# SamGalanakis/FlowCompare

Measured on NVIDIA B200. Metric: cloud-pairs/sec for per-point log p(x|ctx), higher is better.
Workload: dtype fp16x3(f32-faithful)

## Files before the change

flowcompare_b200/csrc/attention_tc.cu:

```cuda
#include <cuda_fp16.h>
#include "common.cuh"
#include "gemm.cuh"
#include "tcgen05.cuh"
#include <atomic>
#include <cstdlib>
#include <mutex>
#include <vector>

namespace {

constexpr int AQ = 128;
constexpr int AK = 64;
constexpr int AD = 64;
#ifndef A_SPL
#define A_SPL 4
#endif
constexpr int A_THREADS = 96 + 128 * A_SPL;
constexpr int A_ATOM = 64 * 128;
constexpr int A_QBYTES = 2 * AQ * 128;
constexpr uint32_t C_S = 128, C_O = 384;
template <bool F16> struct ACfg {
    static constexpr int TILE = F16 ? 2 * A_ATOM : 4 * A_ATOM;
    static constexpr int STAGES = F16 ? 4 : 2;
    static constexpr int SMEM = A_QBYTES + 2 * STAGES * TILE + 1024;
    static constexpr uint32_t C_QHI = 0, C_QLO = F16 ? 32 : 64, C_PHI = 256, C_PLO = F16 ? 288 : 320;
};
constexpr float A_QS = 16.0f;

struct AttnTcParams {
    float* out; int ldo;
    int N, Nc, nblk;
    float scale;
    int debug;
    int dbg_loads;
};

__device__ __forceinline__ void tmem_st16(uint32_t taddr, const uint32_t* r) {
    asm volatile(
        "tcgen05.st.sync.aligned.32x32b.x16.b32 [%0], {%1,%2,%3,%4,%5,%6,%7,%8,%9,%10,%11,%12,%13,%14,%15,%16};"
        ::"r"(taddr), "r"(r[0]), "r"(r[1]), "r"(r[2]), "r"(r[3]), "r"(r[4]), "r"(r[5]), "r"(r[6]), "r"(r[7]), "r"(r[8]),
          "r"(r[9]), "r"(r[10]), "r"(r[11]), "r"(r[12]), "r"(r[13]), "r"(r[14]), "r"(r[15]) : "memory");
}
__device__ __forceinline__ void tmem_st8(uint32_t taddr, const uint32_t* r) {
    asm volatile(
        "tcgen05.st.sync.aligned.32x32b.x8.b32 [%0], {%1,%2,%3,%4,%5,%6,%7,%8};"
        ::"r"(taddr), "r"(r[0]), "r"(r[1]), "r"(r[2]), "r"(r[3]), "r"(r[4]), "r"(r[5]), "r"(r[6]), "r"(r[7]) : "memory");
}
__device__ __forceinline__ float ex2_approx(float x) {
    float y;
    asm("ex2.approx.ftz.f32 %0, %1;" : "=f"(y) : "f"(x));
    return y;
}
__device__ __forceinline__ uint32_t tf32_hi(float x) { return (__float_as_uint(x) + 0x1000u) & 0xffffe000u; }

__device__ __forceinline__ void issue_3xtf32(uint32_t d, uint32_t a_hi, uint32_t a_lo, const unsigned char* b_tile, uint32_t idesc) {
#pragma unroll
    for (int kk = 0; kk < 8; ++kk) {
        const uint32_t atom = (uint32_t)(kk >> 2) * A_ATOM;
        const uint64_t adv = (uint64_t)((kk & 3) * 32 >> 4);
        const uint64_t dbh = make_kmajor_sw128_desc(smem_u32(b_tile + atom)) + adv;
        const uint64_t dbl = make_kmajor_sw128_desc(smem_u32(b_tile + 2 * A_ATOM + atom)) + adv;
        umma_tf32_ts(d, a_lo + 8 * kk, dbh, idesc, kk != 0);
        umma_tf32_ts(d, a_hi + 8 * kk, dbl, idesc, 1);
        umma_tf32_ts(d, a_hi + 8 * kk, dbh, idesc, 1);
    }
}

__device__ __forceinline__ void issue_3xf16(uint32_t d, uint32_t a_hi, uint32_t a_lo, const unsigned char* b_tile, uint32_t idesc) {
#pragma unroll
    for (int kk = 0; kk < 4; ++kk) {
        const uint64_t adv = (uint64_t)(kk * 32 >> 4);
        const uint64_t dbh = make_kmajor_sw128_desc(smem_u32(b_tile)) + adv;
        const uint64_t dbl = make_kmajor_sw128_desc(smem_u32(b_tile + A_ATOM)) + adv;
        umma_f16_ts(d, a_lo + 8 * kk, dbh, idesc, kk != 0);
        umma_f16_ts(d, a_hi + 8 * kk, dbl, idesc, 1);
        umma_f16_ts(d, a_hi + 8 * kk, dbh, idesc, 1);
    }
}

__device__ unsigned long long fc_attn_dbg[16];
#ifndef A_PHASE_TIMERS
#define A_PHASE_TIMERS 0
#endif
#if A_PHASE_TIMERS
#define DBG_T(var) const long long var = p.debug ? clock64() : 0
#else
#define DBG_T(var) const long long var = 0
#endif

template <bool F16>
__global__ void __launch_bounds__(A_THREADS, 1)
attention_tc_kernel(const __grid_constant__ CUtensorMap mapQ, const __grid_constant__ CUtensorMap mapKhi,
                    const __grid_constant__ CUtensorMap mapKlo, const __grid_constant__ CUtensorMap mapVhi,
                    const __grid_constant__ CUtensorMap mapVlo, const AttnTcParams p) {
    constexpr int A_STAGES = ACfg<F16>::STAGES, A_TILE = ACfg<F16>::TILE;
    constexpr uint32_t C_QHI = ACfg<F16>::C_QHI, C_QLO = ACfg<F16>::C_QLO, C_PHI = ACfg<F16>::C_PHI, C_PLO = ACfg<F16>::C_PLO;
    static_assert(!F16 || A_SPL == 2 || A_SPL == 4, "the fp16 form packs 32 (16) dims / keys per thread into one 16 (8) column store");
    extern __shared__ unsigned char smem_raw[];
    __shared__ __align__(8) uint64_t bars[2 + 4 * A_STAGES + 12];
    __shared__ uint32_t tmem_base_slot;
    __shared__ float mx_sm[2][A_SPL][AQ];

    const uint32_t raw = smem_u32(smem_raw);
    unsigned char* smem = smem_raw + ((1024u - (raw & 1023u)) & 1023u);
    unsigned char* q_raw = smem;
    auto k_tile = [&](int s) { return smem + A_QBYTES + s * A_TILE; };
    auto v_tile = [&](int s) { return smem + A_QBYTES + (A_STAGES + s) * A_TILE; };
    uint64_t* qfull = bars;
    uint64_t* qready = bars + 1;
    uint64_t* kfull = bars + 2;
    uint64_t* kfree = kfull + A_STAGES;
    uint64_t* vfull = kfree + A_STAGES;
    uint64_t* vfree = vfull + A_STAGES;
    uint64_t* s_ready = vfree + A_STAGES;
    uint64_t* s_free = s_ready + 2;
    constexpr int NPB = F16 ? 2 : 1;
    uint64_t* p_ready = s_free + 2;
    uint64_t* p_free = p_ready + 2;
    uint64_t* o_ready = p_free + 2;
    uint64_t* o_free = o_ready + 2;

    const int warp = threadIdx.x >> 5, lane = threadIdx.x & 31;
    const int b = blockIdx.y;
    const int q0 = blockIdx.x * AQ;
    const int nblk = p.nblk;

    if (threadIdx.x == 0) {
        mbar_init(qfull, 1); mbar_init(qready, 128 * A_SPL);
        for (int s = 0; s < A_STAGES; ++s) { mbar_init(&kfull[s], 1); mbar_init(&kfree[s], 1); mbar_init(&vfull[s], 1); mbar_init(&vfree[s], 1); }
        for (int s = 0; s < 2; ++s) { mbar_init(&s_ready[s], 1); mbar_init(&s_free[s], 128 * A_SPL); mbar_init(&o_ready[s], 1); mbar_init(&o_free[s], 128 * A_SPL); }
        for (int s = 0; s < 2; ++s) { mbar_init(&p_ready[s], 128 * A_SPL); mbar_init(&p_free[s], 1); }
        asm volatile("fence.mbarrier_init.release.cluster;" ::: "memory");
    }
    if (warp == 1) {
        asm volatile("tcgen05.alloc.cta_group::1.sync.aligned.shared::cta.b32 [%0], %1;" ::"r"(smem_u32(&tmem_base_slot)), "n"(512));
        asm volatile("tcgen05.relinquish_alloc_permit.cta_group::1.sync.aligned;");
    }
    asm volatile("tcgen05.fence::before_thread_sync;" ::: "memory");
    __syncthreads();
    asm volatile("tcgen05.fence::after_thread_sync;" ::: "memory");
    const uint32_t tmem = tmem_base_slot;

    if (warp == 0) {
        if (lane == 0) {
            mbar_expect_tx(qfull, A_QBYTES);
            tma_load_2d(&mapQ, q_raw, qfull, 0, b * p.N + q0);
            tma_load_2d(&mapQ, q_raw + AQ * 128, qfull, 32, b * p.N + q0);
            for (int i = 0; i < nblk; ++i) {
                const int s = i % A_STAGES;
                const uint32_t ph = (i / A_STAGES) & 1;
                const int krow = b * p.Nc + i * AK;
                mbar_wait(&kfree[s], ph ^ 1, 100 + i);
                if constexpr (F16) {
                    mbar_expect_tx(&kfull[s], A_TILE);
                    tma_load_2d(&mapKhi, k_tile(s), &kfull[s], 0, krow);
                    tma_load_2d(&mapKlo, k_tile(s) + A_ATOM, &kfull[s], 0, krow);
                    mbar_wait(&vfree[s], ph ^ 1, 150 + i);
                    mbar_expect_tx(&vfull[s], A_TILE);
                    tma_load_3d(&mapVhi, v_tile(s), &vfull[s], i * AK, 0, b);
                    tma_load_3d(&mapVlo, v_tile(s) + A_ATOM, &vfull[s], i * AK, 0, b);
                } else {
                mbar_expect_tx(&kfull[s], p.dbg_loads ? A_TILE / 2 : A_TILE);
                tma_load_2d(&mapKhi, k_tile(s), &kfull[s], 0, krow);
                tma_load_2d(&mapKhi, k_tile(s) + A_ATOM, &kfull[s], 32, krow);
                if (!p.dbg_loads) {
                tma_load_2d(&mapKlo, k_tile(s) + 2 * A_ATOM, &kfull[s], 0, krow);
                tma_load_2d(&mapKlo, k_tile(s) + 3 * A_ATOM, &kfull[s], 32, krow);
                }
                mbar_wait(&vfree[s], ph ^ 1, 150 + i);
                mbar_expect_tx(&vfull[s], p.dbg_loads ? A_TILE / 2 : A_TILE);
                tma_load_3d(&mapVhi, v_tile(s), &vfull[s], i * AK, 0, b);
                tma_load_3d(&mapVhi, v_tile(s) + A_ATOM, &vfull[s], i * AK + 32, 0, b);
                if (!p.dbg_loads) {
                tma_load_3d(&mapVlo, v_tile(s) + 2 * A_ATOM, &vfull[s], i * AK, 0, b);
                tma_load_3d(&mapVlo, v_tile(s) + 3 * A_ATOM, &vfull[s], i * AK + 32, 0, b);
                }
                }
            }
        }
    } else if (warp == 1) {
        const uint32_t idesc = (1u << 4) | ((F16 ? 0u : 2u) << 7) | ((F16 ? 0u : 2u) << 10) | ((uint32_t)(AK >> 3) << 17) | ((uint32_t)(AQ >> 4) << 24);
        long long w_kfull = 0, w_sfree = 0;
        DBG_T(t_start);
        mbar_wait(qready, 0, 200);
        asm volatile("tcgen05.fence::after_thread_sync;" ::: "memory");
        DBG_T(t_q);
        for (int j = 0; j < nblk; ++j) {
            const int ks = j % A_STAGES, sb = j & 1;
            DBG_T(c0);
            mbar_wait(&kfull[ks], (j / A_STAGES) & 1, 210 + j);
            DBG_T(c1);
            mbar_wait(&s_free[sb], ((j >> 1) & 1) ^ 1, 220 + j);
            DBG_T(c2);
            w_kfull += c1 - c0; w_sfree += c2 - c1;
            asm volatile("tcgen05.fence::after_thread_sync;" ::: "memory");
            if (elect_one()) {
                if constexpr (F16) issue_3xf16(tmem + C_S + 64 * sb, tmem + C_QHI, tmem + C_QLO, k_tile(ks), idesc);
                else issue_3xtf32(tmem + C_S + 64 * sb, tmem + C_QHI, tmem + C_QLO, k_tile(ks), idesc);
                umma_commit(&s_ready[sb]);
                umma_commit(&kfree[ks]);
            }
            __syncwarp();
        }
        if (A_PHASE_TIMERS && p.debug && lane == 0) {
            atomicAdd(&fc_attn_dbg[0], 1ull);
            atomicAdd(&fc_attn_dbg[1], (unsigned long long)(clock64() - t_start));
            atomicAdd(&fc_attn_dbg[2], (unsigned long long)w_kfull); atomicAdd(&fc_attn_dbg[3], (unsigned long long)w_sfree);
            atomicAdd(&fc_attn_dbg[11], (unsigned long long)(t_q - t_start));
        }
    } else if (warp == 2) {
        const uint32_t idesc = (1u << 4) | ((F16 ? 0u : 2u) << 7) | ((F16 ? 0u : 2u) << 10) | ((uint32_t)(AK >> 3) << 17) | ((uint32_t)(AQ >> 4) << 24);
        long long w_vfull = 0, w_ofree = 0, w_pready = 0;
        for (int i = 0; i < nblk; ++i) {
            const int vs = i % A_STAGES, ob = i & 1;
            DBG_T(c3);
            mbar_wait(&vfull[vs], (i / A_STAGES) & 1, 230 + i);
            DBG_T(c4);
            mbar_wait(&o_free[ob], ((i >> 1) & 1) ^ 1, 240 + i);
            DBG_T(c5);
            const int pb = NPB == 2 ? (i & 1) : 0;
            mbar_wait(&p_ready[pb], NPB == 2 ? (i >> 1) & 1 : i & 1, 250 + i);
            DBG_T(c6);
            w_vfull += c4 - c3; w_ofree += c5 - c4; w_pready += c6 - c5;
            asm volatile("tcgen05.fence::after_thread_sync;" ::: "memory");
            if (elect_one()) {
                if constexpr (F16) issue_3xf16(tmem + C_O + 64 * ob, tmem + C_PHI + 64 * pb, tmem + C_PLO + 64 * pb, v_tile(vs), idesc);
                else issue_3xtf32(tmem + C_O + 64 * ob, tmem + C_PHI, tmem + C_PLO, v_tile(vs), idesc);
                umma_commit(&o_ready[ob]);
                umma_commit(&p_free[pb]);
                umma_commit(&vfree[vs]);
            }
            __syncwarp();
        }
        if (A_PHASE_TIMERS && p.debug && lane == 0) {
            atomicAdd(&fc_attn_dbg[4], (unsigned long long)w_vfull); atomicAdd(&fc_attn_dbg[5], (unsigned long long)w_ofree);
            atomicAdd(&fc_attn_dbg[6], (unsigned long long)w_pready);
        }
    } else {
        constexpr int KS = AK / A_SPL;
        const int quad = warp & 3;
        const int sub = (warp - 3) >> 2;
        const int r = quad * 32 + lane;
        const uint32_t lane_addr = (uint32_t)(quad * 32) << 16;
        const int off = sub * KS;
        const float LOG2E = F16 ? 1.4426950408889634f / A_QS : 1.4426950408889634f;
        const int bar_id = 1 + quad;

        mbar_wait(qfull, 0, 300);
        if constexpr (F16) {
            uint32_t hi[KS / 2], lo[KS / 2];
            const unsigned char* atom = q_raw + (off >> 5) * (AQ * 128) + r * 128;
            const int j0 = (off & 31) >> 2;
            const float qs = p.scale * A_QS;
#pragma unroll
            for (int j = 0; j < KS / 4; ++j) {
                const float4 x = *reinterpret_cast<const float4*>(atom + (((j0 + j) ^ (r & 7)) << 4));
                const float xv[4] = {x.x * qs, x.y * qs, x.z * qs, x.w * qs};
#pragma unroll
                for (int e = 0; e < 4; e += 2) {
                    const uint32_t hp = pack_f16x2(xv[e], xv[e + 1]);
                    float h0, h1;
                    unpack_f16x2(hp, h0, h1);
                    hi[2 * j + (e >> 1)] = hp;
                    lo[2 * j + (e >> 1)] = pack_f16x2(xv[e] - h0, xv[e + 1] - h1);
                }
            }
            if constexpr (KS == 32) { tmem_st16(tmem + lane_addr + C_QHI + (off >> 1), hi); tmem_st16(tmem + lane_addr + C_QLO + (off >> 1), lo); }
            else                    { tmem_st8(tmem + lane_addr + C_QHI + (off >> 1), hi);  tmem_st8(tmem + lane_addr + C_QLO + (off >> 1), lo); }
        } else
#pragma unroll
        for (int c = 0; c < KS / 16; ++c) {
            uint32_t hi[16], lo[16];
            const int d0 = off + 16 * c;
            const unsigned char* atom = q_raw + (d0 >> 5) * (AQ * 128) + r * 128;
#pragma unroll
            for (int jj = 0; jj < 4; ++jj) {
                const int j = ((d0 & 31) >> 2) + jj;
                const float4 x = *reinterpret_cast<const float4*>(atom + ((j ^ (r & 7)) << 4));
                const float xv[4] = {x.x * p.scale, x.y * p.scale, x.z * p.scale, x.w * p.scale};
#pragma unroll
                for (int e = 0; e < 4; ++e) {
                    hi[4 * jj + e] = tf32_hi(xv[e]);
                    lo[4 * jj + e] = __float_as_uint(xv[e] - __uint_as_float(hi[4 * jj + e]));
                }
            }
            tmem_st16(tmem + lane_addr + C_QHI + d0, hi);
            tmem_st16(tmem + lane_addr + C_QLO + d0, lo);
        }
        asm volatile("tcgen05.wait::st.sync.aligned;" ::: "memory");
        asm volatile("tcgen05.fence::before_thread_sync;" ::: "memory");
        mbar_arrive(qready);

        float o[KS];
#pragma unroll
        for (int j = 0; j < KS; ++j) o[j] = 0.f;
        float m = -INFINITY, l = 0.f, alpha_prev = 0.f;

        auto load_cols = [&](uint32_t col, float (&dst)[KS]) {
#pragma unroll
            for (int c = 0; c < KS / 16; ++c) {
                uint32_t t16[16];
                tmem_ld16(tmem + lane_addr + col + 16 * c, t16);
#pragma unroll
                for (int j = 0; j < 16; ++j) dst[16 * c + j] = __uint_as_float(t16[j]);
            }
        };

        long long w_sready = 0, w_pfree = 0, w_oready = 0;
        DBG_T(t_sm0);
        for (int i = 0; i < nblk; ++i) {
            const int sb = i & 1;
            float sv[KS];
            DBG_T(d0);
            mbar_wait(&s_ready[sb], (i >> 1) & 1, 310 + i);
            DBG_T(d1);
            w_sready += d1 - d0;
            asm volatile("tcgen05.fence::after_thread_sync;" ::: "memory");
            load_cols(C_S + 64 * sb + off, sv);
            asm volatile("tcgen05.fence::before_thread_sync;" ::: "memory");
            mbar_arrive(&s_free[sb]);
            const int valid = p.Nc - i * AK - off;
            if (valid < KS) {
#pragma unroll
                for (int j = 0; j < KS; ++j) if (j >= valid) sv[j] = -INFINITY;
            }
            float mx4[4] = {sv[0], sv[1], sv[2], sv[3]};
#pragma unroll
            for (int j = 4; j < KS; ++j) mx4[j & 3] = fmaxf(mx4[j & 3], sv[j]);
            float mx = fmaxf(fmaxf(mx4[0], mx4[1]), fmaxf(mx4[2], mx4[3]));
            if (A_SPL > 1) {
                mx_sm[sb][sub][r] = mx;
                asm volatile("bar.sync %0, %1;" ::"r"(bar_id), "n"(32 * A_SPL) : "memory");
#pragma unroll
                for (int u = 0; u < A_SPL; ++u) mx = fmaxf(mx, mx_sm[sb][u][r]);
            }
            const float m_new = fmaxf(m, mx);
            const float alpha = ex2_approx((m - m_new) * LOG2E);
            const float mc = F16 ? fmaf(m_new, LOG2E, -10.0f) : m_new * LOG2E;
            float sum4[4] = {0.f, 0.f, 0.f, 0.f};
#pragma unroll
            for (int j = 0; j < KS; j += 4) {
                const float2 t0 = __ffma2_rn(make_float2(sv[j], sv[j + 1]), make_float2(LOG2E, LOG2E), make_float2(-mc, -mc));
                const float2 t1 = __ffma2_rn(make_float2(sv[j + 2], sv[j + 3]), make_float2(LOG2E, LOG2E), make_float2(-mc, -mc));
                sv[j] = ex2_approx(t0.x); sv[j + 1] = ex2_approx(t0.y); sv[j + 2] = ex2_approx(t1.x); sv[j + 3] = ex2_approx(t1.y);
                const float2 s01 = __fadd2_rn(make_float2(sum4[0], sum4[1]), make_float2(sv[j], sv[j + 1]));
                const float2 s23 = __fadd2_rn(make_float2(sum4[2], sum4[3]), make_float2(sv[j + 2], sv[j + 3]));
                sum4[0] = s01.x; sum4[1] = s01.y; sum4[2] = s23.x; sum4[3] = s23.y;
            }
            l = fmaf(l, alpha, (sum4[0] + sum4[1]) + (sum4[2] + sum4[3]));
            m = m_new;

            DBG_T(d2);
            const int pb = NPB == 2 ? (i & 1) : 0;
            mbar_wait(&p_free[pb], (NPB == 2 ? (i >> 1) & 1 : i & 1) ^ 1, 330 + i);
            DBG_T(d3);
            w_pfree += d3 - d2;
            asm volatile("tcgen05.fence::after_thread_sync;" ::: "memory");
            if constexpr (F16) {
                uint32_t hi[KS / 2], lo[KS / 2];
#pragma unroll
                for (int j = 0; j < KS / 2; ++j) {
                    const float p0 = sv[2 * j], p1 = sv[2 * j + 1];
                    const uint32_t hp = pack_f16x2(p0, p1);
                    float h0, h1;
                    unpack_f16x2(hp, h0, h1);
                    hi[j] = hp;
                    const float2 d2 = __fadd2_rn(make_float2(p0, p1), make_float2(-h0, -h1));
                    lo[j] = pack_f16x2(d2.x, d2.y);
                }
                if constexpr (KS == 32) { tmem_st16(tmem + lane_addr + C_PHI + 64 * pb + (off >> 1), hi); tmem_st16(tmem + lane_addr + C_PLO + 64 * pb + (off >> 1), lo); }
                else                    { tmem_st8(tmem + lane_addr + C_PHI + 64 * pb + (off >> 1), hi);  tmem_st8(tmem + lane_addr + C_PLO + 64 * pb + (off >> 1), lo); }
            } else
#pragma unroll
            for (int c = 0; c < KS / 16; ++c) {
                uint32_t hi[16], lo[16];
#pragma unroll
                for (int j = 0; j < 16; ++j) {
                    hi[j] = tf32_hi(sv[16 * c + j]);
                    lo[j] = __float_as_uint(sv[16 * c + j] - __uint_as_float(hi[j]));
                }
                tmem_st16(tmem + lane_addr + C_PHI + off + 16 * c, hi);
                tmem_st16(tmem + lane_addr + C_PLO + off + 16 * c, lo);
            }
            asm volatile("tcgen05.wait::st.sync.aligned;" ::: "memory");
            asm volatile("tcgen05.fence::before_thread_sync;" ::: "memory");
            mbar_arrive(&p_ready[pb]);

            if (i > 0) {
                const int ob = (i - 1) & 1;
                float ov[KS];
                DBG_T(d4);
                mbar_wait(&o_ready[ob], ((i - 1) >> 1) & 1, 350 + i);
                DBG_T(d5);
                w_oready += d5 - d4;
                asm volatile("tcgen05.fence::after_thread_sync;" ::: "memory");
                load_cols(C_O + 64 * ob + off, ov);
                asm volatile("tcgen05.fence::before_thread_sync;" ::: "memory");
                mbar_arrive(&o_free[ob]);
#pragma unroll
                for (int j = 0; j < KS; j += 2) {
                    const float2 o2 = __ffma2_rn(make_float2(o[j], o[j + 1]), make_float2(alpha_prev, alpha_prev), make_float2(ov[j], ov[j + 1]));
                    o[j] = o2.x; o[j + 1] = o2.y;
                }
            }
            alpha_prev = alpha;
        }
        if (A_PHASE_TIMERS && p.debug && threadIdx.x == 96) {
            atomicAdd(&fc_attn_dbg[7], (unsigned long long)w_sready); atomicAdd(&fc_attn_dbg[8], (unsigned long long)w_pfree);
            atomicAdd(&fc_attn_dbg[9], (unsigned long long)w_oready); atomicAdd(&fc_attn_dbg[10], (unsigned long long)(clock64() - t_sm0));
        }
        {
            const int ob = (nblk - 1) & 1;
            float ov[KS];
            mbar_wait(&o_ready[ob], ((nblk - 1) >> 1) & 1, 390);
            asm volatile("tcgen05.fence::after_thread_sync;" ::: "memory");
            load_cols(C_O + 64 * ob + off, ov);
#pragma unroll
            for (int j = 0; j < KS; ++j) o[j] = fmaf(o[j], alpha_prev, ov[j]);
        }
        if (A_SPL > 1) {
            mx_sm[nblk & 1][sub][r] = l;
            asm volatile("bar.sync %0, %1;" ::"r"(bar_id), "n"(32 * A_SPL) : "memory");
            l = 0.f;
#pragma unroll
            for (int u = 0; u < A_SPL; ++u) l += mx_sm[nblk & 1][u][r];
        }
        if (q0 + r < p.N) {
            const float inv = 1.0f / l;
            float4* dst = reinterpret_cast<float4*>(p.out + ((size_t)b * p.N + q0 + r) * p.ldo + off);
#pragma unroll
            for (int j = 0; j < KS / 4; ++j)
                dst[j] = make_float4(o[4 * j] * inv, o[4 * j + 1] * inv, o[4 * j + 2] * inv, o[4 * j + 3] * inv);
        }
    }
    asm volatile("tcgen05.fence::before_thread_sync;" ::: "memory");
    __syncthreads();
    if (warp == 1) {
        asm volatile("tcgen05.dealloc.cta_group::1.sync.aligned.b32 %0, %1;" ::"r"(tmem), "n"(512));
    }
}

template <bool F16>
__global__ void __launch_bounds__(256)
kv_split_kernel(const float* __restrict__ kv, int ldkv, int Nc, int Ncp, void* __restrict__ khi_, void* __restrict__ klo_,
                void* __restrict__ vthi_, void* __restrict__ vtlo_) {
    __shared__ float tile[32][AD + 1];
    const int b = blockIdx.y, key0 = blockIdx.x * 32, tid = threadIdx.x;
    auto put = [](void* hi_, void* lo_, size_t i, float x) {
        if (F16) {
            const __half h = __float2half_rn(x);
            static_cast<__half*>(hi_)[i] = h;
            static_cast<__half*>(lo_)[i] = __float2half_rn(x - __half2float(h));
        } else {
            const float h = __uint_as_float(tf32_hi(x));
            static_cast<float*>(hi_)[i] = h;
            static_cast<float*>(lo_)[i] = x - h;
        }
    };
    for (int idx = tid; idx < 32 * AD; idx += 256) {
        const int kk = idx >> 6, d = idx & 63;
        const int key = key0 + kk;
        if (key < Nc) {
            const float* src = kv + ((size_t)b * Nc + key) * ldkv;
            put(khi_, klo_, ((size_t)b * Nc + key) * AD + d, src[d]);
            tile[kk][d] = src[AD + d];
        } else {
            tile[kk][d] = 0.f;
        }
    }
    __syncthreads();
    for (int idx = tid; idx < 32 * AD; idx += 256) {
        const int d = idx >> 5, kk = idx & 31;
        const int key = key0 + kk;
        if (key < Ncp) put(vthi_, vtlo_, ((size_t)b * AD + d) * Ncp + key, tile[kk][d]);
    }
}

struct AMapKey {
    const void* base; uint64_t d0, d1, d2, s1, s2; uint32_t b0, b1; int f16;
    bool operator==(const AMapKey& o) const {
        return base == o.base && d0 == o.d0 && d1 == o.d1 && d2 == o.d2 && s1 == o.s1 && s2 == o.s2 && b0 == o.b0 && b1 == o.b1 && f16 == o.f16;
    }
};
std::vector<std::pair<AMapKey, CUtensorMap>> g_amaps;
std::mutex g_amaps_mu;

bool get_amap(const void* base, uint64_t d0, uint64_t d1, uint64_t d2, uint64_t s1, uint64_t s2, uint32_t b0, uint32_t b1,
              CUtensorMap* out, int f16 = 0) {
    AMapKey key{base, d0, d1, d2, s1, s2, b0, b1, f16};
    std::lock_guard<std::mutex> lk(g_amaps_mu);
    for (auto& kv : g_amaps) if (kv.first == key) { *out = kv.second; return true; }
    FcEncodeTiledFn enc = fc_get_encode_fn();
    if (!enc) return false;
    const cuuint32_t rank = d2 > 0 ? 3 : 2;
    cuuint64_t dims[3] = {d0, d1, d2 > 0 ? d2 : 1};
    const cuuint64_t esz = f16 ? 2 : 4;
    cuuint64_t strides[2] = {s1 * esz, s2 * esz};
    cuuint32_t box[3] = {b0, b1, 1};
    cuuint32_t estr[3] = {1, 1, 1};
    CUtensorMap m;
    if (enc(&m, f16 ? CU_TENSOR_MAP_DATA_TYPE_FLOAT16 : CU_TENSOR_MAP_DATA_TYPE_FLOAT32, rank, const_cast<void*>(base), dims, strides, box, estr,
            CU_TENSOR_MAP_INTERLEAVE_NONE, CU_TENSOR_MAP_SWIZZLE_128B, CU_TENSOR_MAP_L2_PROMOTION_L2_128B,
            CU_TENSOR_MAP_FLOAT_OOB_FILL_NONE) != CUDA_SUCCESS)
        return false;
    if (g_amaps.size() > 256) g_amaps.clear();
    g_amaps.emplace_back(key, m);
    *out = m;
    return true;
}

}

int64_t fc_attention_tc_scratch_floats(int B, int Nc) {
    const int64_t Ncp = fc_round_up(Nc, 8);
    return 2 * fc_round_up_ll((int64_t)B * Nc * AD, 32) + 2 * fc_round_up_ll((int64_t)B * AD * Ncp, 32) + 64;
}

void fc_attention_tc_scratch_layout(int B, int Nc, float* scratch, float** khi, float** klo, float** vthi, float** vtlo,
                                    int* ncp, int fmt) {
    const int Ncp = fc_round_up(Nc, fmt ? 8 : 4);
    *khi = scratch;
    *klo = *khi + fc_round_up_ll((int64_t)B * Nc * AD, 32);
    *vthi = *klo + fc_round_up_ll((int64_t)B * Nc * AD, 32);
    *vtlo = *vthi + fc_round_up_ll((int64_t)B * AD * fc_round_up(Nc, 8), 32);
    *ncp = Ncp;
}

namespace {
template <bool F16>
int launch_attention_tc(const float* q, int ldq, const float* kv, int ldkv, float* out, int ldo, int B, int N, int Nc, int d,
                        float scale, float* scratch, int presplit, cudaStream_t stream) {
    float *khi, *klo, *vthi, *vtlo;
    int Ncp;
    fc_attention_tc_scratch_layout(B, Nc, scratch, &khi, &klo, &vthi, &vtlo, &Ncp, F16 ? 1 : 0);
    CUtensorMap mQ, mKh, mKl, mVh, mVl;
    if (!get_amap(q, AD, (uint64_t)B * N, 0, (uint64_t)ldq, 0, 32, AQ, &mQ)) return FC_ERR_CUDA;
    const uint32_t bx = F16 ? 64 : 32;
    if (!get_amap(khi, AD, (uint64_t)B * Nc, 0, AD, 0, bx, AK, &mKh, F16)) return FC_ERR_CUDA;
    if (!get_amap(klo, AD, (uint64_t)B * Nc, 0, AD, 0, bx, AK, &mKl, F16)) return FC_ERR_CUDA;
    if (!get_amap(vthi, (uint64_t)Nc, AD, (uint64_t)B, (uint64_t)Ncp, (uint64_t)AD * Ncp, bx, AD, &mVh, F16)) return FC_ERR_CUDA;
    if (!get_amap(vtlo, (uint64_t)Nc, AD, (uint64_t)B, (uint64_t)Ncp, (uint64_t)AD * Ncp, bx, AD, &mVl, F16)) return FC_ERR_CUDA;
    int dev = 0;
    FC_CUDA_OK(cudaGetDevice(&dev));
    static std::atomic<uint64_t> configured{0};
    const uint64_t bit = 1ull << (dev & 63);
    if (!(configured.load(std::memory_order_acquire) & bit)) {
        FC_CUDA_OK(cudaFuncSetAttribute(attention_tc_kernel<F16>, cudaFuncAttributeMaxDynamicSharedMemorySize, ACfg<F16>::SMEM));
        configured.fetch_or(bit, std::memory_order_release);
    }
    FcProfScope prof(FC_CLS_ATTENTION, 4.0 * B * (double)N * Nc * d, 4.0 * B * ((double)N * d * 2 + (double)Nc * d * 2), stream);
    if (!presplit) {
        kv_split_kernel<F16><<<dim3((Ncp + 31) / 32, B), 256, 0, stream>>>(kv, ldkv, Nc, Ncp, khi, klo, vthi, vtlo);
        fc_count_launch();
    }
    static int dbg_loads = -1;
    if (dbg_loads < 0) { const char* e = getenv("FC_ATTN_DBG_LOADS"); dbg_loads = (e && e[0] == '1') ? 1 : 0; }
    static int dbg = -1;
    if (dbg < 0) { const char* e = getenv("FC_ATTN_DEBUG"); dbg = (e && e[0] == '1') ? 1 : 0; }
    AttnTcParams p{out, ldo, N, Nc, (Nc + AK - 1) / AK, scale, dbg, dbg_loads};
    attention_tc_kernel<F16><<<dim3((N + AQ - 1) / AQ, B), A_THREADS, ACfg<F16>::SMEM, stream>>>(mQ, mKh, mKl, mVh, mVl, p);
    fc_count_launch();
    FC_LAUNCH_OK();
    return FC_OK;
}
}

int fc_launch_cross_attention_tc(const float* q, int ldq, const float* kv, int ldkv, float* out, int ldo, int B, int N,
                                 int Nc, int d, float scale, float* scratch, int presplit, int fmt, cudaStream_t stream) {
    FC_REQUIRE(q && (kv || presplit) && out && scratch && B > 0 && N > 0 && Nc > 0);
    FC_REQUIRE((int64_t)B * N < (1ll << 31) - AQ && (int64_t)B * Nc < (1ll << 31) - AK);
    if (d != AD) return FC_ERR_UNSUPPORTED;
    FC_REQUIRE((ldq & 3) == 0 && (ldo & 3) == 0 && (presplit || ldkv >= 2 * AD) && ldq >= AD && ldo >= AD && B <= 65535);
    FC_REQUIRE((reinterpret_cast<uintptr_t>(q) & 15) == 0 && (reinterpret_cast<uintptr_t>(out) & 15) == 0 &&
               (reinterpret_cast<uintptr_t>(scratch) & 127) == 0);
    return fmt ? launch_attention_tc<true>(q, ldq, kv, ldkv, out, ldo, B, N, Nc, d, scale, scratch, presplit, stream)
               : launch_attention_tc<false>(q, ldq, kv, ldkv, out, ldo, B, N, Nc, d, scale, scratch, presplit, stream);
}

extern "C" __attribute__((visibility("default"))) int fc_debug_attn_phases(unsigned long long* out16) {
    if (cudaMemcpyFromSymbol(out16, fc_attn_dbg, 16 * sizeof(unsigned long long)) != cudaSuccess) return FC_ERR_CUDA;
    unsigned long long z[16] = {};
    if (cudaMemcpyToSymbol(fc_attn_dbg, z, sizeof(z)) != cudaSuccess) return FC_ERR_CUDA;
    return FC_OK;
}

extern "C" __attribute__((visibility("default"))) int64_t fc_cross_attention_tc_scratch_bytes(int B, int Nc) {
    if (B <= 0 || Nc <= 0) return FC_ERR_INVALID_ARG;
    return fc_attention_tc_scratch_floats(B, Nc) * 4;
}

extern "C" __attribute__((visibility("default"))) int fc_cross_attention_tc(const float* q, int ldq, const float* kv, int ldkv,
                                                                             float* out, int ldo, int B, int N, int Nc, int d,
                                                                             float scale, void* scratch, int64_t scratch_bytes,
                                                                             fc_stream_t stream) {
    FC_REQUIRE(scratch && scratch_bytes >= fc_cross_attention_tc_scratch_bytes(B, Nc));
    return fc_launch_cross_attention_tc(q, ldq, kv, ldkv, out, ldo, B, N, Nc, d, scale, static_cast<float*>(scratch), 0, 0,
                                        (cudaStream_t)stream);
}

extern "C" __attribute__((visibility("default"))) int fc_cross_attention_tc_f16(const float* q, int ldq, const float* kv, int ldkv,
                                                                                 float* out, int ldo, int B, int N, int Nc, int d,
                                                                                 float scale, void* scratch, int64_t scratch_bytes,
                                                                                 fc_stream_t stream) {
    FC_REQUIRE(scratch && scratch_bytes >= fc_cross_attention_tc_scratch_bytes(B, Nc));
    return fc_launch_cross_attention_tc(q, ldq, kv, ldkv, out, ldo, B, N, Nc, d, scale, static_cast<float*>(scratch), 0, 1,
                                        (cudaStream_t)stream);
}
```

flowcompare_b200/csrc/tcgen05.cuh:

```cuda
#pragma once
#include <cuda.h>
#include <cuda_runtime.h>
#include <cstdint>
#include <cstdio>

namespace {

__device__ __forceinline__ uint32_t smem_u32(const void* p) { return (uint32_t)__cvta_generic_to_shared(p); }

__device__ __forceinline__ void mbar_init(uint64_t* bar, uint32_t count) {
    asm volatile("mbarrier.init.shared::cta.b64 [%0], %1;" ::"r"(smem_u32(bar)), "r"(count));
}
__device__ __forceinline__ void mbar_expect_tx(uint64_t* bar, uint32_t bytes) {
    asm volatile("mbarrier.arrive.expect_tx.shared::cta.b64 _, [%0], %1;" ::"r"(smem_u32(bar)), "r"(bytes) : "memory");
}
__device__ __forceinline__ void mbar_arrive(uint64_t* bar) {
    asm volatile("mbarrier.arrive.shared::cta.b64 _, [%0];" ::"r"(smem_u32(bar)) : "memory");
}
__device__ __forceinline__ void mbar_timeout(int tag, uint32_t parity) {
    printf("flowcompare_b200 tcgen05 kernel: mbarrier wait timed out (tag %d, block %d,%d thread %d, parity %u)\n", tag,
           blockIdx.x, blockIdx.y, threadIdx.x, parity);
    __trap();
}
__device__ __forceinline__ void mbar_wait(uint64_t* bar, uint32_t parity, int tag = 0) {
    uint32_t done = 0;
    for (uint32_t spin = 0; spin < (1u << 22); ++spin) {
        asm volatile(
            "{\n\t"
            ".reg .pred p;\n\t"
            "mbarrier.try_wait.parity.shared::cta.b64 p, [%1], %2;\n\t"
            "selp.u32 %0, 1, 0, p;\n\t"
            "}" : "=r"(done) : "r"(smem_u32(bar)), "r"(parity) : "memory");
        if (done) return;
    }
    mbar_timeout(tag, parity);
}
__device__ __forceinline__ void mbar_wait_hint(uint64_t* bar, uint32_t parity, int tag, uint32_t hint_ns) {
    if (hint_ns == 0) { mbar_wait(bar, parity, tag); return; }
    uint32_t done = 0;
    for (uint32_t spin = 0; spin < (1u << 22); ++spin) {
        asm volatile(
            "{\n\t"
            ".reg .pred p;\n\t"
            "mbarrier.try_wait.parity.shared::cta.b64 p, [%1], %2, %3;\n\t"
            "selp.u32 %0, 1, 0, p;\n\t"
            "}" : "=r"(done) : "r"(smem_u32(bar)), "r"(parity), "r"(hint_ns) : "memory");
        if (done) return;
    }
    mbar_timeout(tag, parity);
}
__device__ __forceinline__ bool mbar_test(uint64_t* bar, uint32_t parity) {
    uint32_t done;
    asm volatile(
        "{\n\t"
        ".reg .pred p;\n\t"
        "mbarrier.test_wait.parity.shared::cta.b64 p, [%1], %2;\n\t"
        "selp.u32 %0, 1, 0, p;\n\t"
        "}" : "=r"(done) : "r"(smem_u32(bar)), "r"(parity) : "memory");
    return done != 0;
}
__device__ __forceinline__ void tma_load_2d(const CUtensorMap* map, void* smem_dst, uint64_t* bar, int c0, int c1) {
    asm volatile(
        "cp.async.bulk.tensor.2d.shared::cluster.global.mbarrier::complete_tx::bytes [%0], [%1, {%3, %4}], [%2];"
        ::"r"(smem_u32(smem_dst)), "l"(map), "r"(smem_u32(bar)), "r"(c0), "r"(c1) : "memory");
}
__device__ __forceinline__ void tma_load_2d_mcast(const CUtensorMap* map, void* smem_dst, uint64_t* bar, int c0, int c1,
                                                  uint16_t mask) {
    asm volatile(
        "cp.async.bulk.tensor.2d.shared::cluster.global.mbarrier::complete_tx::bytes.multicast::cluster"
        " [%0], [%1, {%3, %4}], [%2], %5;"
        ::"r"(smem_u32(smem_dst)), "l"(map), "r"(smem_u32(bar)), "r"(c0), "r"(c1), "h"(mask) : "memory");
}
__device__ __forceinline__ void tma_store_2d(const CUtensorMap* map, const void* smem_src, int c0, int c1) {
    asm volatile("cp.async.bulk.tensor.2d.global.shared::cta.bulk_group [%0, {%2, %3}], [%1];"
                 ::"l"(map), "r"(smem_u32(smem_src)), "r"(c0), "r"(c1) : "memory");
}
__device__ __forceinline__ void umma_commit(uint64_t* bar) {
    asm volatile("tcgen05.commit.cta_group::1.mbarrier::arrive::one.shared::cluster.b64 [%0];" ::"r"(smem_u32(bar)) : "memory");
}
__device__ __forceinline__ void umma_commit_mcast(uint64_t* bar, uint16_t mask) {
    asm volatile("tcgen05.commit.cta_group::1.mbarrier::arrive::one.shared::cluster.multicast::cluster.b64 [%0], %1;"
                 ::"r"(smem_u32(bar)), "h"(mask) : "memory");
}
__device__ __forceinline__ bool elect_one() {
    uint32_t pred;
    asm volatile("{\n\t.reg .b32 rx;\n\t.reg .pred px;\n\telect.sync rx|px, 0xffffffff;\n\tselp.u32 %0, 1, 0, px;\n\t}" : "=r"(pred));
    return pred != 0;
}
__device__ __forceinline__ void cluster_sync_all() {
    asm volatile("barrier.cluster.arrive.release.aligned;\n\tbarrier.cluster.wait.acquire.aligned;" ::: "memory");
}
__device__ __forceinline__ void umma_tf32_ts(uint32_t tmem_d, uint32_t tmem_a, uint64_t desc_b, uint32_t idesc, uint32_t accumulate) {
    #if !(defined(TC_KO_MMA) && TC_KO_MMA)
    asm volatile(
        "{\n\t"
        ".reg .pred p;\n\t"
        "setp.ne.b32 p, %4, 0;\n\t"
        "tcgen05.mma.cta_group::1.kind::tf32 [%0], [%1], %2, %3, p;\n\t"
        "}" ::"r"(tmem_d), "r"(tmem_a), "l"(desc_b), "r"(idesc), "r"(accumulate) : "memory");
#endif
}
__device__ __forceinline__ void umma_f16_ts(uint32_t tmem_d, uint32_t tmem_a, uint64_t desc_b, uint32_t idesc, uint32_t accumulate) {
    #if !(defined(TC_KO_MMA) && TC_KO_MMA)
    asm volatile(
        "{\n\t"
        ".reg .pred p;\n\t"
        "setp.ne.b32 p, %4, 0;\n\t"
        "tcgen05.mma.cta_group::1.kind::f16 [%0], [%1], %2, %3, p;\n\t"
        "}" ::"r"(tmem_d), "r"(tmem_a), "l"(desc_b), "r"(idesc), "r"(accumulate) : "memory");
#endif
}
__device__ __forceinline__ uint64_t make_kmajor_sw64_desc(uint32_t smem_addr) {
    uint64_t d = 0;
    d |= (uint64_t)((smem_addr & 0x3FFFF) >> 4);
    d |= (uint64_t)1 << 16;
    d |= (uint64_t)(512 >> 4) << 32;
    d |= (uint64_t)1 << 46;
    d |= (uint64_t)4 << 61;
    return d;
}
__device__ __forceinline__ uint32_t pack_f16x2(float lo_half, float hi_half) {
    uint32_t r;
    asm("cvt.rn.f16x2.f32 %0, %1, %2;" : "=r"(r) : "f"(hi_half), "f"(lo_half));
    return r;
}
__device__ __forceinline__ void unpack_f16x2(uint32_t v, float& lo_half, float& hi_half) {
    asm("{\n\t.reg .f16 l, h;\n\tmov.b32 {l, h}, %2;\n\tcvt.f32.f16 %0, l;\n\tcvt.f32.f16 %1, h;\n\t}" : "=f"(lo_half), "=f"(hi_half) : "r"(v));
}
__device__ __forceinline__ uint64_t make_kmajor_sw128_desc(uint32_t smem_addr) {
    uint64_t d = 0;
    d |= (uint64_t)((smem_addr & 0x3FFFF) >> 4);
    d |= (uint64_t)1 << 16;
    d |= (uint64_t)(1024 >> 4) << 32;
    d |= (uint64_t)1 << 46;
    d |= (uint64_t)2 << 61;
    return d;
}
__device__ __forceinline__ void tmem_ld16(uint32_t taddr, uint32_t (&r)[16]) {
    asm volatile(
        "tcgen05.ld.sync.aligned.32x32b.x16.b32 {%0,%1,%2,%3,%4,%5,%6,%7,%8,%9,%10,%11,%12,%13,%14,%15}, [%16];\n\t"
        "tcgen05.wait::ld.sync.aligned;"
        : "=r"(r[0]), "=r"(r[1]), "=r"(r[2]), "=r"(r[3]), "=r"(r[4]), "=r"(r[5]), "=r"(r[6]), "=r"(r[7]), "=r"(r[8]),
          "=r"(r[9]), "=r"(r[10]), "=r"(r[11]), "=r"(r[12]), "=r"(r[13]), "=r"(r[14]), "=r"(r[15])
        : "r"(taddr) : "memory");
}
__device__ __forceinline__ void tmem_ld16x2(uint32_t taddr_a, uint32_t taddr_b, uint32_t (&a)[16], uint32_t (&b)[16]) {
    asm volatile(
        "tcgen05.ld.sync.aligned.32x32b.x16.b32 {%0,%1,%2,%3,%4,%5,%6,%7,%8,%9,%10,%11,%12,%13,%14,%15}, [%32];\n\t"
        "tcgen05.ld.sync.aligned.32x32b.x16.b32 {%16,%17,%18,%19,%20,%21,%22,%23,%24,%25,%26,%27,%28,%29,%30,%31}, [%33];\n\t"
        "tcgen05.wait::ld.sync.aligned;"
        : "=r"(a[0]), "=r"(a[1]), "=r"(a[2]), "=r"(a[3]), "=r"(a[4]), "=r"(a[5]), "=r"(a[6]), "=r"(a[7]), "=r"(a[8]),
          "=r"(a[9]), "=r"(a[10]), "=r"(a[11]), "=r"(a[12]), "=r"(a[13]), "=r"(a[14]), "=r"(a[15]),
          "=r"(b[0]), "=r"(b[1]), "=r"(b[2]), "=r"(b[3]), "=r"(b[4]), "=r"(b[5]), "=r"(b[6]), "=r"(b[7]), "=r"(b[8]),
          "=r"(b[9]), "=r"(b[10]), "=r"(b[11]), "=r"(b[12]), "=r"(b[13]), "=r"(b[14]), "=r"(b[15])
        : "r"(taddr_a), "r"(taddr_b) : "memory");
}
__device__ __forceinline__ void tmem_ld16x2_issue(uint32_t taddr_a, uint32_t taddr_b, uint32_t (&a)[16], uint32_t (&b)[16]) {
    asm volatile(
        "tcgen05.ld.sync.aligned.32x32b.x16.b32 {%0,%1,%2,%3,%4,%5,%6,%7,%8,%9,%10,%11,%12,%13,%14,%15}, [%32];\n\t"
        "tcgen05.ld.sync.aligned.32x32b.x16.b32 {%16,%17,%18,%19,%20,%21,%22,%23,%24,%25,%26,%27,%28,%29,%30,%31}, [%33];"
        : "=r"(a[0]), "=r"(a[1]), "=r"(a[2]), "=r"(a[3]), "=r"(a[4]), "=r"(a[5]), "=r"(a[6]), "=r"(a[7]), "=r"(a[8]),
          "=r"(a[9]), "=r"(a[10]), "=r"(a[11]), "=r"(a[12]), "=r"(a[13]), "=r"(a[14]), "=r"(a[15]),
          "=r"(b[0]), "=r"(b[1]), "=r"(b[2]), "=r"(b[3]), "=r"(b[4]), "=r"(b[5]), "=r"(b[6]), "=r"(b[7]), "=r"(b[8]),
          "=r"(b[9]), "=r"(b[10]), "=r"(b[11]), "=r"(b[12]), "=r"(b[13]), "=r"(b[14]), "=r"(b[15])
        : "r"(taddr_a), "r"(taddr_b) : "memory");
}
__device__ __forceinline__ void tmem_ld16x2_wait(uint32_t (&a)[16], uint32_t (&b)[16]) {
    asm volatile("tcgen05.wait::ld.sync.aligned;"
        : "+r"(a[0]), "+r"(a[1]), "+r"(a[2]), "+r"(a[3]), "+r"(a[4]), "+r"(a[5]), "+r"(a[6]), "+r"(a[7]), "+r"(a[8]),
          "+r"(a[9]), "+r"(a[10]), "+r"(a[11]), "+r"(a[12]), "+r"(a[13]), "+r"(a[14]), "+r"(a[15]),
          "+r"(b[0]), "+r"(b[1]), "+r"(b[2]), "+r"(b[3]), "+r"(b[4]), "+r"(b[5]), "+r"(b[6]), "+r"(b[7]), "+r"(b[8]),
          "+r"(b[9]), "+r"(b[10]), "+r"(b[11]), "+r"(b[12]), "+r"(b[13]), "+r"(b[14]), "+r"(b[15])
        :: "memory");
}
__device__ __forceinline__ void tmem_st16(uint32_t taddr, const uint32_t (&r)[16]) {
    asm volatile(
        "tcgen05.st.sync.aligned.32x32b.x16.b32 [%0], {%1,%2,%3,%4,%5,%6,%7,%8,%9,%10,%11,%12,%13,%14,%15,%16};"
        ::"r"(taddr), "r"(r[0]), "r"(r[1]), "r"(r[2]), "r"(r[3]), "r"(r[4]), "r"(r[5]), "r"(r[6]), "r"(r[7]), "r"(r[8]),
          "r"(r[9]), "r"(r[10]), "r"(r[11]), "r"(r[12]), "r"(r[13]), "r"(r[14]), "r"(r[15]) : "memory");
}
__device__ __forceinline__ void tmem_st32(uint32_t taddr, const uint32_t (&r)[32]) {
    asm volatile(
        "tcgen05.st.sync.aligned.32x32b.x32.b32 [%0], {%1,%2,%3,%4,%5,%6,%7,%8,%9,%10,%11,%12,%13,%14,%15,%16,"
        "%17,%18,%19,%20,%21,%22,%23,%24,%25,%26,%27,%28,%29,%30,%31,%32};"
        ::"r"(taddr), "r"(r[0]), "r"(r[1]), "r"(r[2]), "r"(r[3]), "r"(r[4]), "r"(r[5]), "r"(r[6]), "r"(r[7]), "r"(r[8]),
          "r"(r[9]), "r"(r[10]), "r"(r[11]), "r"(r[12]), "r"(r[13]), "r"(r[14]), "r"(r[15]), "r"(r[16]), "r"(r[17]),
          "r"(r[18]), "r"(r[19]), "r"(r[20]), "r"(r[21]), "r"(r[22]), "r"(r[23]), "r"(r[24]), "r"(r[25]), "r"(r[26]),
          "r"(r[27]), "r"(r[28]), "r"(r[29]), "r"(r[30]), "r"(r[31]) : "memory");
}

__device__ __forceinline__ void tmem_ld32(uint32_t taddr, uint32_t (&r)[32]) {
    asm volatile(
        "tcgen05.ld.sync.aligned.32x32b.x32.b32 {%0,%1,%2,%3,%4,%5,%6,%7,%8,%9,%10,%11,%12,%13,%14,%15,%16,%17,%18,%19,%20,"
        "%21,%22,%23,%24,%25,%26,%27,%28,%29,%30,%31}, [%32];\n\t"
        "tcgen05.wait::ld.sync.aligned;"
        : "=r"(r[0]), "=r"(r[1]), "=r"(r[2]), "=r"(r[3]), "=r"(r[4]), "=r"(r[5]), "=r"(r[6]), "=r"(r[7]), "=r"(r[8]),
          "=r"(r[9]), "=r"(r[10]), "=r"(r[11]), "=r"(r[12]), "=r"(r[13]), "=r"(r[14]), "=r"(r[15]), "=r"(r[16]), "=r"(r[17]),
          "=r"(r[18]), "=r"(r[19]), "=r"(r[20]), "=r"(r[21]), "=r"(r[22]), "=r"(r[23]), "=r"(r[24]), "=r"(r[25]), "=r"(r[26]),
          "=r"(r[27]), "=r"(r[28]), "=r"(r[29]), "=r"(r[30]), "=r"(r[31])
        : "r"(taddr) : "memory");
}
__device__ __forceinline__ void tma_load_3d(const CUtensorMap* map, void* smem_dst, uint64_t* bar, int c0, int c1, int c2) {
    asm volatile(
        "cp.async.bulk.tensor.3d.shared::cluster.global.mbarrier::complete_tx::bytes [%0], [%1, {%3, %4, %5}], [%2];"
        ::"r"(smem_u32(smem_dst)), "l"(map), "r"(smem_u32(bar)), "r"(c0), "r"(c1), "r"(c2) : "memory");
}

typedef CUresult (*FcEncodeTiledFn)(CUtensorMap*, CUtensorMapDataType, cuuint32_t, void*, const cuuint64_t*, const cuuint64_t*,
                                    const cuuint32_t*, const cuuint32_t*, CUtensorMapInterleave, CUtensorMapSwizzle,
                                    CUtensorMapL2promotion, CUtensorMapFloatOOBfill);
inline FcEncodeTiledFn fc_get_encode_fn() {
    static FcEncodeTiledFn fn = nullptr;
    static bool tried = false;
    if (!tried) {
        tried = true;
        void* p = nullptr;
        cudaDriverEntryPointQueryResult q;
        if (cudaGetDriverEntryPoint("cuTensorMapEncodeTiled", &p, cudaEnableDefault, &q) == cudaSuccess &&
            q == cudaDriverEntryPointSuccess)
            fn = reinterpret_cast<FcEncodeTiledFn>(p);
    }
    return fn;
}

}
```

Before: 531.1.

## Split fp16 attention into dedicated kernel with 128-key blocks and SS MMA

Replaces the templated attention kernel with separate tf32 and fp16 kernels. The fp16 path gets a new kernel that processes 128 keys per block, keeps Q in shared memory for SS-form MMAs, aliases S and P in TMEM, and uses a cheaper bit-trick fp16 hi split plus an optional polynomial exp2. The aim is to halve the per-block barrier and softmax sync overhead and shorten the MMA critical path. The cost is more shared memory per stage, more registers per softmax thread, and a large new code path that may carry correctness risk.

```diff
diff --git a/flowcompare_b200/csrc/attention_tc.cu b/flowcompare_b200/csrc/attention_tc.cu
--- a/flowcompare_b200/csrc/attention_tc.cu
+++ b/flowcompare_b200/csrc/attention_tc.cu
@@ -11,6 +11,7 @@
 
 constexpr int AQ = 128;
 constexpr int AK = 64;
+constexpr int FK = 128;
 constexpr int AD = 64;
 #ifndef A_SPL
 #define A_SPL 4
@@ -18,13 +19,12 @@
 constexpr int A_THREADS = 96 + 128 * A_SPL;
 constexpr int A_ATOM = 64 * 128;
 constexpr int A_QBYTES = 2 * AQ * 128;
-constexpr uint32_t C_S = 128, C_O = 384;
-template <bool F16> struct ACfg {
-    static constexpr int TILE = F16 ? 2 * A_ATOM : 4 * A_ATOM;
-    static constexpr int STAGES = F16 ? 4 : 2;
-    static constexpr int SMEM = A_QBYTES + 2 * STAGES * TILE + 1024;
-    static constexpr uint32_t C_QHI = 0, C_QLO = F16 ? 32 : 64, C_PHI = 256, C_PLO = F16 ? 288 : 320;
-};
+constexpr int T_TILE = 4 * A_ATOM, T_STAGES = 2;
+constexpr int T_SMEM = A_QBYTES + 2 * T_STAGES * T_TILE + 1024;
+constexpr uint32_t T_QHI = 0, T_QLO = 64, C_S = 128, T_PHI = 256, T_PLO = 320, C_O = 384;
+constexpr int F_QTILE = AQ * 128, F_KTILE = 2 * FK * 128, F_VTILE = (FK / 64) * 2 * A_ATOM, F_STAGES = 2;
+constexpr int F_SMEM = A_QBYTES + 2 * F_QTILE + F_STAGES * (F_KTILE + F_VTILE) + 1024;
+constexpr uint32_t F_SP = 0, F_O = 256;
 constexpr float A_QS = 16.0f;
 
 struct AttnTcParams {
@@ -41,15 +41,35 @@
         ::"r"(taddr), "r"(r[0]), "r"(r[1]), "r"(r[2]), "r"(r[3]), "r"(r[4]), "r"(r[5]), "r"(r[6]), "r"(r[7]), "r"(r[8]),
           "r"(r[9]), "r"(r[10]), "r"(r[11]), "r"(r[12]), "r"(r[13]), "r"(r[14]), "r"(r[15]) : "memory");
 }
-__device__ __forceinline__ void tmem_st8(uint32_t taddr, const uint32_t* r) {
-    asm volatile(
-        "tcgen05.st.sync.aligned.32x32b.x8.b32 [%0], {%1,%2,%3,%4,%5,%6,%7,%8};"
-        ::"r"(taddr), "r"(r[0]), "r"(r[1]), "r"(r[2]), "r"(r[3]), "r"(r[4]), "r"(r[5]), "r"(r[6]), "r"(r[7]) : "memory");
-}
 __device__ __forceinline__ float ex2_approx(float x) {
     float y;
     asm("ex2.approx.ftz.f32 %0, %1;" : "=f"(y) : "f"(x));
     return y;
+}
+__device__ __forceinline__ uint32_t p_hi_bits(float p) { return max(__float_as_uint(p) >> 13, 0x1C400u) - 0x1C000u; }
+__device__ __forceinline__ float f16_bits_value(uint32_t h) { return __uint_as_float((h << 13) + 0x38000000u); }
+#ifndef A_EX2_POLY
+#define A_EX2_POLY 0
+#endif
+__device__ __forceinline__ float exp2_poly_scale(float q, float t, float x) {
+    const int n = (int)(__float_as_uint(t) - __float_as_uint(12582912.f));
+    const float r = n < -125 ? 0.f : __uint_as_float(__float_as_uint(q) + ((uint32_t)n << 23));
+    return x != x ? x : r;
+}
+__device__ __forceinline__ float2 exp2_poly2(float2 x) {
+    const float M = 12582912.f;
+    const float2 xc = make_float2(x.x < -127.f ? -127.f : x.x, x.y < -127.f ? -127.f : x.y);
+    const float2 t = __fadd2_rn(xc, make_float2(M, M));
+    const float2 rn = __fadd2_rn(t, make_float2(-M, -M));
+    const float2 f = __fadd2_rn(xc, make_float2(-rn.x, -rn.y));
+    float2 q = make_float2(1.5403530393381608e-4f, 1.5403530393381608e-4f);
+    q = __ffma2_rn(q, f, make_float2(1.3333558146428443e-3f, 1.3333558146428443e-3f));
+    q = __ffma2_rn(q, f, make_float2(9.6181291076284772e-3f, 9.6181291076284772e-3f));
+    q = __ffma2_rn(q, f, make_float2(5.5504108664821580e-2f, 5.5504108664821580e-2f));
+    q = __ffma2_rn(q, f, make_float2(2.4022650695910071e-1f, 2.4022650695910071e-1f));
+    q = __ffma2_rn(q, f, make_float2(6.9314718055994531e-1f, 6.9314718055994531e-1f));
+    q = __ffma2_rn(q, f, make_float2(1.f, 1.f));
+    return make_float2(exp2_poly_scale(q.x, t.x, x.x), exp2_poly_scale(q.y, t.y, x.y));
 }
 __device__ __forceinline__ uint32_t tf32_hi(float x) { return (__float_as_uint(x) + 0x1000u) & 0xffffe000u; }
 
@@ -63,18 +83,6 @@
         umma_tf32_ts(d, a_lo + 8 * kk, dbh, idesc, kk != 0);
         umma_tf32_ts(d, a_hi + 8 * kk, dbl, idesc, 1);
         umma_tf32_ts(d, a_hi + 8 * kk, dbh, idesc, 1);
-    }
-}
-
-__device__ __forceinline__ void issue_3xf16(uint32_t d, uint32_t a_hi, uint32_t a_lo, const unsigned char* b_tile, uint32_t idesc) {
-#pragma unroll
-    for (int kk = 0; kk < 4; ++kk) {
-        const uint64_t adv = (uint64_t)(kk * 32 >> 4);
-        const uint64_t dbh = make_kmajor_sw128_desc(smem_u32(b_tile)) + adv;
-        const uint64_t dbl = make_kmajor_sw128_desc(smem_u32(b_tile + A_ATOM)) + adv;
-        umma_f16_ts(d, a_lo + 8 * kk, dbh, idesc, kk != 0);
-        umma_f16_ts(d, a_hi + 8 * kk, dbl, idesc, 1);
-        umma_f16_ts(d, a_hi + 8 * kk, dbh, idesc, 1);
     }
 }
 
@@ -88,14 +96,11 @@
 #define DBG_T(var) const long long var = 0
 #endif
 
-template <bool F16>
 __global__ void __launch_bounds__(A_THREADS, 1)
-attention_tc_kernel(const __grid_constant__ CUtensorMap mapQ, const __grid_constant__ CUtensorMap mapKhi,
-                    const __grid_constant__ CUtensorMap mapKlo, const __grid_constant__ CUtensorMap mapVhi,
-                    const __grid_constant__ CUtensorMap mapVlo, const AttnTcParams p) {
-    constexpr int A_STAGES = ACfg<F16>::STAGES, A_TILE = ACfg<F16>::TILE;
-    constexpr uint32_t C_QHI = ACfg<F16>::C_QHI, C_QLO = ACfg<F16>::C_QLO, C_PHI = ACfg<F16>::C_PHI, C_PLO = ACfg<F16>::C_PLO;
-    static_assert(!F16 || A_SPL == 2 || A_SPL == 4, "the fp16 form packs 32 (16) dims / keys per thread into one 16 (8) column store");
+attention_tc_tf32_kernel(const __grid_constant__ CUtensorMap mapQ, const __grid_constant__ CUtensorMap mapKhi,
+                         const __grid_constant__ CUtensorMap mapKlo, const __grid_constant__ CUtensorMap mapVhi,
+                         const __grid_constant__ CUtensorMap mapVlo, const AttnTcParams p) {
+    constexpr int A_STAGES = T_STAGES, A_TILE = T_TILE;
     extern __shared__ unsigned char smem_raw[];
     __shared__ __align__(8) uint64_t bars[2 + 4 * A_STAGES + 12];
     __shared__ uint32_t tmem_base_slot;
@@ -114,7 +119,6 @@
     uint64_t* vfree = vfull + A_STAGES;
     uint64_t* s_ready = vfree + A_STAGES;
     uint64_t* s_free = s_ready + 2;
-    constexpr int NPB = F16 ? 2 : 1;
     uint64_t* p_ready = s_free + 2;
     uint64_t* p_free = p_ready + 2;
     uint64_t* o_ready = p_free + 2;
@@ -151,15 +155,6 @@
                 const uint32_t ph = (i / A_STAGES) & 1;
                 const int krow = b * p.Nc + i * AK;
                 mbar_wait(&kfree[s], ph ^ 1, 100 + i);
-                if constexpr (F16) {
-                    mbar_expect_tx(&kfull[s], A_TILE);
-                    tma_load_2d(&mapKhi, k_tile(s), &kfull[s], 0, krow);
-                    tma_load_2d(&mapKlo, k_tile(s) + A_ATOM, &kfull[s], 0, krow);
-                    mbar_wait(&vfree[s], ph ^ 1, 150 + i);
-                    mbar_expect_tx(&vfull[s], A_TILE);
-                    tma_load_3d(&mapVhi, v_tile(s), &vfull[s], i * AK, 0, b);
-                    tma_load_3d(&mapVlo, v_tile(s) + A_ATOM, &vfull[s], i * AK, 0, b);
-                } else {
                 mbar_expect_tx(&kfull[s], p.dbg_loads ? A_TILE / 2 : A_TILE);
                 tma_load_2d(&mapKhi, k_tile(s), &kfull[s], 0, krow);
                 tma_load_2d(&mapKhi, k_tile(s) + A_ATOM, &kfull[s], 32, krow);
@@ -175,11 +170,10 @@
                 tma_load_3d(&mapVlo, v_tile(s) + 2 * A_ATOM, &vfull[s], i * AK, 0, b);
                 tma_load_3d(&mapVlo, v_tile(s) + 3 * A_ATOM, &vfull[s], i * AK + 32, 0, b);
                 }
-                }
             }
         }
     } else if (warp == 1) {
-        const uint32_t idesc = (1u << 4) | ((F16 ? 0u : 2u) << 7) | ((F16 ? 0u : 2u) << 10) | ((uint32_t)(AK >> 3) << 17) | ((uint32_t)(AQ >> 4) << 24);
+        const uint32_t idesc = (1u << 4) | (2u << 7) | (2u << 10) | ((uint32_t)(AK >> 3) << 17) | ((uint32_t)(AQ >> 4) << 24);
         long long w_kfull = 0, w_sfree = 0;
         DBG_T(t_start);
         mbar_wait(qready, 0, 200);
@@ -195,8 +189,7 @@
             w_kfull += c1 - c0; w_sfree += c2 - c1;
             asm volatile("tcgen05.fence::after_thread_sync;" ::: "memory");
             if (elect_one()) {
-                if constexpr (F16) issue_3xf16(tmem + C_S + 64 * sb, tmem + C_QHI, tmem + C_QLO, k_tile(ks), idesc);
-                else issue_3xtf32(tmem + C_S + 64 * sb, tmem + C_QHI, tmem + C_QLO, k_tile(ks), idesc);
+                issue_3xtf32(tmem + C_S + 64 * sb, tmem + T_QHI, tmem + T_QLO, k_tile(ks), idesc);
                 umma_commit(&s_ready[sb]);
                 umma_commit(&kfree[ks]);
             }
@@ -207,10 +200,12 @@
             atomicAdd(&fc_attn_dbg[1], (unsigned long long)(clock64() - t_start));
             atomicAdd(&fc_attn_dbg[2], (unsigned long long)w_kfull); atomicAdd(&fc_attn_dbg[3], (unsigned long long)w_sfree);
             atomicAdd(&fc_attn_dbg[11], (unsigned long long)(t_q - t_start));
+            atomicAdd(&fc_attn_dbg[13], (unsigned long long)nblk);
         }
     } else if (warp == 2) {
-        const uint32_t idesc = (1u << 4) | ((F16 ? 0u : 2u) << 7) | ((F16 ? 0u : 2u) << 10) | ((uint32_t)(AK >> 3) << 17) | ((uint32_t)(AQ >> 4) << 24);
+        const uint32_t idesc = (1u << 4) | (2u << 7) | (2u << 10) | ((uint32_t)(AK >> 3) << 17) | ((uint32_t)(AQ >> 4) << 24);
         long long w_vfull = 0, w_ofree = 0, w_pready = 0;
+        DBG_T(t_pv0);
         for (int i = 0; i < nblk; ++i) {
             const int vs = i % A_STAGES, ob = i & 1;
             DBG_T(c3);
@@ -218,16 +213,14 @@
             DBG_T(c4);
             mbar_wait(&o_free[ob], ((i >> 1) & 1) ^ 1, 240 + i);
             DBG_T(c5);
-            const int pb = NPB == 2 ? (i & 1) : 0;
-            mbar_wait(&p_ready[pb], NPB == 2 ? (i >> 1) & 1 : i & 1, 250 + i);
+            mbar_wait(&p_ready[0], i & 1, 250 + i);
             DBG_T(c6);
             w_vfull += c4 - c3; w_ofree += c5 - c4; w_pready += c6 - c5;
             asm volatile("tcgen05.fence::after_thread_sync;" ::: "memory");
             if (elect_one()) {
-                if constexpr (F16) issue_3xf16(tmem + C_O + 64 * ob, tmem + C_PHI + 64 * pb, tmem + C_PLO + 64 * pb, v_tile(vs), idesc);
-                else issue_3xtf32(tmem + C_O + 64 * ob, tmem + C_PHI, tmem + C_PLO, v_tile(vs), idesc);
+                issue_3xtf32(tmem + C_O + 64 * ob, tmem + T_PHI, tmem + T_PLO, v_tile(vs), idesc);
                 umma_commit(&o_ready[ob]);
-                umma_commit(&p_free[pb]);
+                umma_commit(&p_free[0]);
                 umma_commit(&vfree[vs]);
             }
             __syncwarp();
@@ -235,6 +228,7 @@
         if (A_PHASE_TIMERS && p.debug && lane == 0) {
             atomicAdd(&fc_attn_dbg[4], (unsigned long long)w_vfull); atomicAdd(&fc_attn_dbg[5], (unsigned long long)w_ofree);
             atomicAdd(&fc_attn_dbg[6], (unsigned long long)w_pready);
+            atomicAdd(&fc_attn_dbg[12], (unsigned long long)(clock64() - t_pv0));
         }
     } else {
         constexpr int KS = AK / A_SPL;
@@ -243,31 +237,10 @@
         const int r = quad * 32 + lane;
         const uint32_t lane_addr = (uint32_t)(quad * 32) << 16;
         const int off = sub * KS;
-        const float LOG2E = F16 ? 1.4426950408889634f / A_QS : 1.4426950408889634f;
+        const float LOG2E = 1.4426950408889634f;
         const int bar_id = 1 + quad;
 
         mbar_wait(qfull, 0, 300);
-        if constexpr (F16) {
-            uint32_t hi[KS / 2], lo[KS / 2];
-            const unsigned char* atom = q_raw + (off >> 5) * (AQ * 128) + r * 128;
-            const int j0 = (off & 31) >> 2;
-            const float qs = p.scale * A_QS;
-#pragma unroll
-            for (int j = 0; j < KS / 4; ++j) {
-                const float4 x = *reinterpret_cast<const float4*>(atom + (((j0 + j) ^ (r & 7)) << 4));
-                const float xv[4] = {x.x * qs, x.y * qs, x.z * qs, x.w * qs};
-#pragma unroll
-                for (int e = 0; e < 4; e += 2) {
-                    const uint32_t hp = pack_f16x2(xv[e], xv[e + 1]);
-                    float h0, h1;
-                    unpack_f16x2(hp, h0, h1);
-                    hi[2 * j + (e >> 1)] = hp;
-                    lo[2 * j + (e >> 1)] = pack_f16x2(xv[e] - h0, xv[e + 1] - h1);
-                }
-            }
-            if constexpr (KS == 32) { tmem_st16(tmem + lane_addr + C_QHI + (off >> 1), hi); tmem_st16(tmem + lane_addr + C_QLO + (off >> 1), lo); }
-            else                    { tmem_st8(tmem + lane_addr + C_QHI + (off >> 1), hi);  tmem_st8(tmem + lane_addr + C_QLO + (off >> 1), lo); }
-        } else
 #pragma unroll
         for (int c = 0; c < KS / 16; ++c) {
             uint32_t hi[16], lo[16];
@@ -284,8 +257,8 @@
                     lo[4 * jj + e] = __float_as_uint(xv[e] - __uint_as_float(hi[4 * jj + e]));
                 }
             }
-            tmem_st16(tmem + lane_addr + C_QHI + d0, hi);
-            tmem_st16(tmem + lane_addr + C_QLO + d0, lo);
+            tmem_st16(tmem + lane_addr + T_QHI + d0, hi);
+            tmem_st16(tmem + lane_addr + T_QLO + d0, lo);
         }
         asm volatile("tcgen05.wait::st.sync.aligned;" ::: "memory");
         asm volatile("tcgen05.fence::before_thread_sync;" ::: "memory");
@@ -336,7 +309,7 @@
             }
             const float m_new = fmaxf(m, mx);
             const float alpha = ex2_approx((m - m_new) * LOG2E);
-            const float mc = F16 ? fmaf(m_new, LOG2E, -10.0f) : m_new * LOG2E;
+            const float mc = m_new * LOG2E;
             float sum4[4] = {0.f, 0.f, 0.f, 0.f};
 #pragma unroll
             for (int j = 0; j < KS; j += 4) {
@@ -351,26 +324,10 @@
             m = m_new;
 
             DBG_T(d2);
-            const int pb = NPB == 2 ? (i & 1) : 0;
-            mbar_wait(&p_free[pb], (NPB == 2 ? (i >> 1) & 1 : i & 1) ^ 1, 330 + i);
+            mbar_wait(&p_free[0], (i & 1) ^ 1, 330 + i);
             DBG_T(d3);
             w_pfree += d3 - d2;
             asm volatile("tcgen05.fence::after_thread_sync;" ::: "memory");
-            if constexpr (F16) {
-                uint32_t hi[KS / 2], lo[KS / 2];
-#pragma unroll
-                for (int j = 0; j < KS / 2; ++j) {
-                    const float p0 = sv[2 * j], p1 = sv[2 * j + 1];
-                    const uint32_t hp = pack_f16x2(p0, p1);
-                    float h0, h1;
-                    unpack_f16x2(hp, h0, h1);
-                    hi[j] = hp;
-                    const float2 d2 = __fadd2_rn(make_float2(p0, p1), make_float2(-h0, -h1));
-                    lo[j] = pack_f16x2(d2.x, d2.y);
-                }
-                if constexpr (KS == 32) { tmem_st16(tmem + lane_addr + C_PHI + 64 * pb + (off >> 1), hi); tmem_st16(tmem + lane_addr + C_PLO + 64 * pb + (off >> 1), lo); }
-                else                    { tmem_st8(tmem + lane_addr + C_PHI + 64 * pb + (off >> 1), hi);  tmem_st8(tmem + lane_addr + C_PLO + 64 * pb + (off >> 1), lo); }
-            } else
 #pragma unroll
             for (int c = 0; c < KS / 16; ++c) {
                 uint32_t hi[16], lo[16];
@@ -379,12 +336,12 @@
                     hi[j] = tf32_hi(sv[16 * c + j]);
                     lo[j] = __float_as_uint(sv[16 * c + j] - __uint_as_float(hi[j]));
                 }
-                tmem_st16(tmem + lane_addr + C_PHI + off + 16 * c, hi);
-                tmem_st16(tmem + lane_addr + C_PLO + off + 16 * c, lo);
+                tmem_st16(tmem + lane_addr + T_PHI + off + 16 * c, hi);
+                tmem_st16(tmem + lane_addr + T_PLO + off + 16 * c, lo);
             }
             asm volatile("tcgen05.wait::st.sync.aligned;" ::: "memory");
             asm volatile("tcgen05.fence::before_thread_sync;" ::: "memory");
-            mbar_arrive(&p_ready[pb]);
+            mbar_arrive(&p_ready[0]);
 
             if (i > 0) {
                 const int ob = (i - 1) & 1;
@@ -430,6 +387,328 @@
             float4* dst = reinterpret_cast<float4*>(p.out + ((size_t)b * p.N + q0 + r) * p.ldo + off);
 #pragma unroll
             for (int j = 0; j < KS / 4; ++j)
+                dst[j] = make_float4(o[4 * j] * inv, o[4 * j + 1] * inv, o[4 * j + 2] * inv, o[4 * j + 3] * inv);
+        }
+    }
+    asm volatile("tcgen05.fence::before_thread_sync;" ::: "memory");
+    __syncthreads();
+    if (warp == 1) {
+        asm volatile("tcgen05.dealloc.cta_group::1.sync.aligned.b32 %0, %1;" ::"r"(tmem), "n"(512));
+    }
+}
+
+__global__ void __launch_bounds__(A_THREADS, 1)
+attention_tc_f16_kernel(const __grid_constant__ CUtensorMap mapQ, const __grid_constant__ CUtensorMap mapKhi,
+                        const __grid_constant__ CUtensorMap mapKlo, const __grid_constant__ CUtensorMap mapVhi,
+                        const __grid_constant__ CUtensorMap mapVlo, const AttnTcParams p) {
+    static_assert(A_SPL == 2 || A_SPL == 4, "the fp16 form gives each softmax thread whole 16-column TMEM loads and stores");
+    extern __shared__ unsigned char smem_raw[];
+    __shared__ __align__(8) uint64_t bars[2 + 4 * F_STAGES + 10];
+    __shared__ uint32_t tmem_base_slot;
+    __shared__ float mx_sm[2][A_SPL][AQ];
+
+    const uint32_t raw = smem_u32(smem_raw);
+    unsigned char* smem = smem_raw + ((1024u - (raw & 1023u)) & 1023u);
+    unsigned char* q_raw = smem;
+    unsigned char* q16 = smem + A_QBYTES;
+    auto k_tile = [&](int s) { return q16 + 2 * F_QTILE + s * F_KTILE; };
+    auto v_tile = [&](int s) { return q16 + 2 * F_QTILE + (F_STAGES * F_KTILE) + s * F_VTILE; };
+    uint64_t* qfull = bars;
+    uint64_t* qready = bars + 1;
+    uint64_t* kfull = bars + 2;
+    uint64_t* kfree = kfull + F_STAGES;
+    uint64_t* vfull = kfree + F_STAGES;
+    uint64_t* vfree = vfull + F_STAGES;
+    uint64_t* s_ready = vfree + F_STAGES;
+    uint64_t* p_ready = s_ready + 2;
+    uint64_t* p_free = p_ready + 2;
+    uint64_t* o_ready = p_free + 2;
+    uint64_t* o_free = o_ready + 2;
+
+    const int warp = threadIdx.x >> 5, lane = threadIdx.x & 31;
+    const int b = blockIdx.y;
+    const int q0 = blockIdx.x * AQ;
+    const int nblk = p.nblk;
+
+    if (threadIdx.x == 0) {
+        mbar_init(qfull, 1); mbar_init(qready, 128 * A_SPL);
+        for (int s = 0; s < F_STAGES; ++s) { mbar_init(&kfull[s], 1); mbar_init(&kfree[s], 1); mbar_init(&vfull[s], 1); mbar_init(&vfree[s], 1); }
+        for (int s = 0; s < 2; ++s) {
+            mbar_init(&s_ready[s], 1); mbar_init(&p_ready[s], 128 * A_SPL); mbar_init(&p_free[s], 1);
+            mbar_init(&o_ready[s], 1); mbar_init(&o_free[s], 128 * A_SPL);
+        }
+        asm volatile("fence.mbarrier_init.release.cluster;" ::: "memory");
+    }
+    if (warp == 1) {
+        asm volatile("tcgen05.alloc.cta_group::1.sync.aligned.shared::cta.b32 [%0], %1;" ::"r"(smem_u32(&tmem_base_slot)), "n"(512));
+        asm volatile("tcgen05.relinquish_alloc_permit.cta_group::1.sync.aligned;");
+    }
+    asm volatile("tcgen05.fence::before_thread_sync;" ::: "memory");
+    __syncthreads();
+    asm volatile("tcgen05.fence::after_thread_sync;" ::: "memory");
+    const uint32_t tmem = tmem_base_slot;
+
+    if (warp == 0) {
+        if (lane == 0) {
+            mbar_expect_tx(qfull, A_QBYTES);
+            tma_load_2d(&mapQ, q_raw, qfull, 0, b * p.N + q0);
+            tma_load_2d(&mapQ, q_raw + AQ * 128, qfull, 32, b * p.N + q0);
+            for (int i = 0; i < nblk; ++i) {
+                const int s = i % F_STAGES;
+                const uint32_t ph = (i / F_STAGES) & 1;
+                const int krow = b * p.Nc + i * FK;
+                mbar_wait(&kfree[s], ph ^ 1, 100 + i);
+                mbar_expect_tx(&kfull[s], F_KTILE);
+                tma_load_2d(&mapKhi, k_tile(s), &kfull[s], 0, krow);
+                tma_load_2d(&mapKlo, k_tile(s) + FK * 128, &kfull[s], 0, krow);
+                mbar_wait(&vfree[s], ph ^ 1, 150 + i);
+                mbar_expect_tx(&vfull[s], F_VTILE);
+#pragma unroll
+                for (int c = 0; c < FK / 64; ++c) {
+                    tma_load_3d(&mapVhi, v_tile(s) + c * 2 * A_ATOM, &vfull[s], i * FK + 64 * c, 0, b);
+                    tma_load_3d(&mapVlo, v_tile(s) + c * 2 * A_ATOM + A_ATOM, &vfull[s], i * FK + 64 * c, 0, b);
+                }
+            }
+        }
+    } else if (warp == 1) {
+        const uint32_t idesc = (1u << 4) | ((uint32_t)(FK >> 3) << 17) | ((uint32_t)(AQ >> 4) << 24);
+        const uint64_t dqh = make_kmajor_sw128_desc(smem_u32(q16)), dql = make_kmajor_sw128_desc(smem_u32(q16 + F_QTILE));
+        long long w_kfull = 0, w_sfree = 0;
+        DBG_T(t_start);
+        mbar_wait(qready, 0, 200);
+        DBG_T(t_q);
+        for (int j = 0; j < nblk; ++j) {
+            const int ks = j % F_STAGES, sb = j & 1;
+            DBG_T(c0);
+            mbar_wait(&kfull[ks], (j / F_STAGES) & 1, 210 + j);
+            DBG_T(c1);
+            mbar_wait(&p_free[sb], ((j >> 1) & 1) ^ 1, 220 + j);
+            DBG_T(c2);
+            w_kfull += c1 - c0; w_sfree += c2 - c1;
+            asm volatile("tcgen05.fence::after_thread_sync;" ::: "memory");
+            if (elect_one()) {
+                const uint64_t dkh = make_kmajor_sw128_desc(smem_u32(k_tile(ks)));
+                const uint64_t dkl = make_kmajor_sw128_desc(smem_u32(k_tile(ks) + FK * 128));
+                const uint32_t d = tmem + F_SP + 128 * sb;
+#pragma unroll
+                for (int kk = 0; kk < AD / 16; ++kk) {
+                    const uint64_t adv = (uint64_t)(kk * 32 >> 4);
+                    umma_f16_ss(d, dql + adv, dkh + adv, idesc, kk != 0);
+                    umma_f16_ss(d, dqh + adv, dkl + adv, idesc, 1);
+                    umma_f16_ss(d, dqh + adv, dkh + adv, idesc, 1);
+                }
+                umma_commit(&s_ready[sb]);
+                umma_commit(&kfree[ks]);
+            }
+            __syncwarp();
+        }
+        if (A_PHASE_TIMERS && p.debug && lane == 0) {
+            atomicAdd(&fc_attn_dbg[0], 1ull);
+            atomicAdd(&fc_attn_dbg[1], (unsigned long long)(clock64() - t_start));
+            atomicAdd(&fc_attn_dbg[2], (unsigned long long)w_kfull); atomicAdd(&fc_attn_dbg[3], (unsigned long long)w_sfree);
+            atomicAdd(&fc_attn_dbg[11], (unsigned long long)(t_q - t_start));
+            atomicAdd(&fc_attn_dbg[13], (unsigned long long)nblk);
+        }
+    } else if (warp == 2) {
+        const uint32_t idesc_w = (1u << 4) | ((uint32_t)(2 * AD >> 3) << 17) | ((uint32_t)(AQ >> 4) << 24);
+        const uint32_t idesc_n = (1u << 4) | ((uint32_t)(AD >> 3) << 17) | ((uint32_t)(AQ >> 4) << 24);
+        long long w_vfull = 0, w_ofree = 0, w_pready = 0;
+        DBG_T(t_pv0);
+        for (int i = 0; i < nblk; ++i) {
+            const int vs = i % F_STAGES, ob = i & 1, sb = i & 1;
+            DBG_T(c3);
+            mbar_wait(&vfull[vs], (i / F_STAGES) & 1, 230 + i);
+            DBG_T(c4);
+            mbar_wait(&o_free[ob], ((i >> 1) & 1) ^ 1, 240 + i);
+            DBG_T(c5);
+            mbar_wait(&p_ready[sb], (i >> 1) & 1, 250 + i);
+            DBG_T(c6);
+            w_vfull += c4 - c3; w_ofree += c5 - c4; w_pready += c6 - c5;
+            asm volatile("tcgen05.fence::after_thread_sync;" ::: "memory");
+            if (elect_one()) {
+                const uint32_t o_main = tmem + F_O + 128 * ob, phi = tmem + F_SP + 128 * sb;
+#pragma unroll
+                for (int kk = 0; kk < FK / 16; ++kk) {
+                    const uint64_t dv = make_kmajor_sw128_desc(smem_u32(v_tile(vs) + (kk >> 2) * 2 * A_ATOM)) + (uint64_t)((kk & 3) * 32 >> 4);
+                    umma_f16_ts(o_main, phi + 8 * kk, dv, idesc_w, kk != 0);
+                    umma_f16_ts(o_main + AD, phi + FK / 2 + 8 * kk, dv, idesc_n, 1);
+                }
+                umma_commit(&o_ready[ob]);
+                umma_commit(&p_free[sb]);
+                umma_commit(&vfree[vs]);
+            }
+            __syncwarp();
+        }
+        if (A_PHASE_TIMERS && p.debug && lane == 0) {
+            atomicAdd(&fc_attn_dbg[4], (unsigned long long)w_vfull); atomicAdd(&fc_attn_dbg[5], (unsigned long long)w_ofree);
+            atomicAdd(&fc_attn_dbg[6], (unsigned long long)w_pready);
+            atomicAdd(&fc_attn_dbg[12], (unsigned long long)(clock64() - t_pv0));
+        }
+    } else {
+        constexpr int KK = FK / A_SPL;
+        constexpr int KD = AD / A_SPL;
+        const int quad = warp & 3;
+        const int sub = (warp - 3) >> 2;
+        const int r = quad * 32 + lane;
+        const uint32_t lane_addr = (uint32_t)(quad * 32) << 16;
+        const int offk = sub * KK, offd = sub * KD;
+        const float LOG2E = 1.4426950408889634f / A_QS;
+        const int bar_id = 1 + quad;
+
+        mbar_wait(qfull, 0, 300);
+        {
+            const unsigned char* atom = q_raw + (offd >> 5) * (AQ * 128) + r * 128;
+            const int j0 = (offd & 31) >> 2;
+            const float qs = p.scale * A_QS;
+#pragma unroll
+            for (int c = 0; c < KD / 8; ++c) {
+                uint32_t hi[4], lo[4];
+#pragma unroll
+                for (int h = 0; h < 2; ++h) {
+                    const float4 x = *reinterpret_cast<const float4*>(atom + (((j0 + 2 * c + h) ^ (r & 7)) << 4));
+                    const float xv[4] = {x.x * qs, x.y * qs, x.z * qs, x.w * qs};
+#pragma unroll
+                    for (int e = 0; e < 4; e += 2) {
+                        const uint32_t hp = pack_f16x2(xv[e], xv[e + 1]);
+                        float h0, h1;
+                        unpack_f16x2(hp, h0, h1);
+                        hi[2 * h + (e >> 1)] = hp;
+                        lo[2 * h + (e >> 1)] = pack_f16x2(xv[e] - h0, xv[e + 1] - h1);
+                    }
+                }
+                const int chunk = ((offd >> 3) + c) ^ (r & 7);
+                *reinterpret_cast<uint4*>(q16 + r * 128 + (chunk << 4)) = make_uint4(hi[0], hi[1], hi[2], hi[3]);
+                *reinterpret_cast<uint4*>(q16 + F_QTILE + r * 128 + (chunk << 4)) = make_uint4(lo[0], lo[1], lo[2], lo[3]);
+            }
+        }
+        asm volatile("fence.proxy.async.shared::cta;" ::: "memory");
+        mbar_arrive(qready);
+
+        float o[KD];
+#pragma unroll
+        for (int j = 0; j < KD; ++j) o[j] = 0.f;
+        float m = -INFINITY, l = 0.f, alpha_prev = 0.f;
+
+        auto fold = [&](uint32_t col, float alpha) {
+#pragma unroll
+            for (int c = 0; c < KD / 16; ++c) {
+                uint32_t om[16], oc[16];
+                tmem_ld16x2(tmem + lane_addr + col + 16 * c, tmem + lane_addr + col + AD + 16 * c, om, oc);
+#pragma unroll
+                for (int j = 0; j < 16; j += 2) {
+                    const float2 s2 = __fadd2_rn(make_float2(__uint_as_float(om[j]), __uint_as_float(om[j + 1])),
+                                                 make_float2(__uint_as_float(oc[j]), __uint_as_float(oc[j + 1])));
+                    const float2 o2 = __ffma2_rn(make_float2(o[16 * c + j], o[16 * c + j + 1]), make_float2(alpha, alpha), s2);
+                    o[16 * c + j] = o2.x; o[16 * c + j + 1] = o2.y;
+                }
+            }
+        };
+
+        long long w_sready = 0, w_oready = 0;
+        DBG_T(t_sm0);
+        for (int i = 0; i < nblk; ++i) {
+            const int sb = i & 1;
+            const uint32_t sp = tmem + lane_addr + F_SP + 128 * sb;
+            float sv[KK];
+            DBG_T(d0);
+            mbar_wait(&s_ready[sb], (i >> 1) & 1, 310 + i);
+            DBG_T(d1);
+            w_sready += d1 - d0;
+            asm volatile("tcgen05.fence::after_thread_sync;" ::: "memory");
+#pragma unroll
+            for (int c = 0; c < KK / 32; ++c) {
+                uint32_t a[16], bb[16];
+                tmem_ld16x2(sp + offk + 32 * c, sp + offk + 32 * c + 16, a, bb);
+#pragma unroll
+                for (int j = 0; j < 16; ++j) { sv[32 * c + j] = __uint_as_float(a[j]); sv[32 * c + 16 + j] = __uint_as_float(bb[j]); }
+            }
+            const int valid = p.Nc - i * FK - offk;
+            if (valid < KK) {
+#pragma unroll
+                for (int j = 0; j < KK; ++j) if (j >= valid) sv[j] = -INFINITY;
+            }
+            float mx4[4] = {sv[0], sv[1], sv[2], sv[3]};
+#pragma unroll
+            for (int j = 4; j < KK; ++j) mx4[j & 3] = fmaxf(mx4[j & 3], sv[j]);
+            float mx = fmaxf(fmaxf(mx4[0], mx4[1]), fmaxf(mx4[2], mx4[3]));
+            mx_sm[sb][sub][r] = mx;
+            asm volatile("tcgen05.fence::before_thread_sync;" ::: "memory");
+            asm volatile("bar.sync %0, %1;" ::"r"(bar_id), "n"(32 * A_SPL) : "memory");
+            asm volatile("tcgen05.fence::after_thread_sync;" ::: "memory");
+#pragma unroll
+            for (int u = 0; u < A_SPL; ++u) mx = fmaxf(mx, mx_sm[sb][u][r]);
+            const float m_new = fmaxf(m, mx);
+            const float alpha = ex2_approx((m - m_new) * LOG2E);
+            const float mc = fmaf(m_new, LOG2E, -10.0f);
+            float sum4[4] = {0.f, 0.f, 0.f, 0.f};
+#pragma unroll
+            for (int j = 0; j < KK; j += 4) {
+                const float2 t0 = __ffma2_rn(make_float2(sv[j], sv[j + 1]), make_float2(LOG2E, LOG2E), make_float2(-mc, -mc));
+                const float2 t1 = __ffma2_rn(make_float2(sv[j + 2], sv[j + 3]), make_float2(LOG2E, LOG2E), make_float2(-mc, -mc));
+                if (A_EX2_POLY && (j & 7) == 4) {
+                    const float2 e01 = exp2_poly2(t0), e23 = exp2_poly2(t1);
+                    sv[j] = e01.x; sv[j + 1] = e01.y; sv[j + 2] = e23.x; sv[j + 3] = e23.y;
+                } else {
+                    sv[j] = ex2_approx(t0.x); sv[j + 1] = ex2_approx(t0.y); sv[j + 2] = ex2_approx(t1.x); sv[j + 3] = ex2_approx(t1.y);
+                }
+                const float2 s01 = __fadd2_rn(make_float2(sum4[0], sum4[1]), make_float2(sv[j], sv[j + 1]));
+                const float2 s23 = __fadd2_rn(make_float2(sum4[2], sum4[3]), make_float2(sv[j + 2], sv[j + 3]));
+                sum4[0] = s01.x; sum4[1] = s01.y; sum4[2] = s23.x; sum4[3] = s23.y;
+            }
+            l = fmaf(l, alpha, (sum4[0] + sum4[1]) + (sum4[2] + sum4[3]));
+            m = m_new;
+
+#pragma unroll
+            for (int c = 0; c < KK / 32; ++c) {
+                uint32_t hi[16], lo[16];
+#pragma unroll
+                for (int j = 0; j < 16; ++j) {
+                    const float p0 = sv[32 * c + 2 * j], p1 = sv[32 * c + 2 * j + 1];
+                    const uint32_t h0 = p_hi_bits(p0), h1 = p_hi_bits(p1);
+                    hi[j] = __byte_perm(h0, h1, 0x5410);
+                    const float2 d2 = __fadd2_rn(make_float2(p0, p1), make_float2(-f16_bits_value(h0), -f16_bits_value(h1)));
+                    lo[j] = pack_f16x2(d2.x, d2.y);
+                }
+                tmem_st16(sp + (offk >> 1) + 16 * c, hi);
+                tmem_st16(sp + FK / 2 + (offk >> 1) + 16 * c, lo);
+            }
+            asm volatile("tcgen05.wait::st.sync.aligned;" ::: "memory");
+            asm volatile("tcgen05.fence::before_thread_sync;" ::: "memory");
+            mbar_arrive(&p_ready[sb]);
+
+            if (i > 0) {
+                const int ob = (i - 1) & 1;
+                DBG_T(d4);
+                mbar_wait(&o_ready[ob], ((i - 1) >> 1) & 1, 350 + i);
+                DBG_T(d5);
+                w_oready += d5 - d4;
+                asm volatile("tcgen05.fence::after_thread_sync;" ::: "memory");
+                fold(F_O + 128 * ob + offd, alpha_prev);
+                asm volatile("tcgen05.fence::before_thread_sync;" ::: "memory");
+                mbar_arrive(&o_free[ob]);
+            }
+            alpha_prev = alpha;
+        }
+        if (A_PHASE_TIMERS && p.debug && threadIdx.x == 96) {
+            atomicAdd(&fc_attn_dbg[7], (unsigned long long)w_sready);
+            atomicAdd(&fc_attn_dbg[9], (unsigned long long)w_oready); atomicAdd(&fc_attn_dbg[10], (unsigned long long)(clock64() - t_sm0));
+        }
+        {
+            const int ob = (nblk - 1) & 1;
+            mbar_wait(&o_ready[ob], ((nblk - 1) >> 1) & 1, 390);
+            asm volatile("tcgen05.fence::after_thread_sync;" ::: "memory");
+            fold(F_O + 128 * ob + offd, alpha_prev);
+        }
+        mx_sm[nblk & 1][sub][r] = l;
+        asm volatile("bar.sync %0, %1;" ::"r"(bar_id), "n"(32 * A_SPL) : "memory");
+        l = 0.f;
+#pragma unroll
+        for (int u = 0; u < A_SPL; ++u) l += mx_sm[nblk & 1][u][r];
+        if (q0 + r < p.N) {
+            const float inv = 1.0f / l;
+            float4* dst = reinterpret_cast<float4*>(p.out + ((size_t)b * p.N + q0 + r) * p.ldo + offd);
+#pragma unroll
+            for (int j = 0; j < KD / 4; ++j)
                 dst[j] = make_float4(o[4 * j] * inv, o[4 * j + 1] * inv, o[4 * j + 2] * inv, o[4 * j + 3] * inv);
         }
     }
@@ -536,16 +815,19 @@
     CUtensorMap mQ, mKh, mKl, mVh, mVl;
     if (!get_amap(q, AD, (uint64_t)B * N, 0, (uint64_t)ldq, 0, 32, AQ, &mQ)) return FC_ERR_CUDA;
     const uint32_t bx = F16 ? 64 : 32;
-    if (!get_amap(khi, AD, (uint64_t)B * Nc, 0, AD, 0, bx, AK, &mKh, F16)) return FC_ERR_CUDA;
-    if (!get_amap(klo, AD, (uint64_t)B * Nc, 0, AD, 0, bx, AK, &mKl, F16)) return FC_ERR_CUDA;
+    const int kblk = F16 ? FK : AK;
+    if (!get_amap(khi, AD, (uint64_t)B * Nc, 0, AD, 0, bx, kblk, &mKh, F16)) return FC_ERR_CUDA;
+    if (!get_amap(klo, AD, (uint64_t)B * Nc, 0, AD, 0, bx, kblk, &mKl, F16)) return FC_ERR_CUDA;
     if (!get_amap(vthi, (uint64_t)Nc, AD, (uint64_t)B, (uint64_t)Ncp, (uint64_t)AD * Ncp, bx, AD, &mVh, F16)) return FC_ERR_CUDA;
     if (!get_amap(vtlo, (uint64_t)Nc, AD, (uint64_t)B, (uint64_t)Ncp, (uint64_t)AD * Ncp, bx, AD, &mVl, F16)) return FC_ERR_CUDA;
     int dev = 0;
     FC_CUDA_OK(cudaGetDevice(&dev));
     static std::atomic<uint64_t> configured{0};
     const uint64_t bit = 1ull << (dev & 63);
+    const int smem = F16 ? F_SMEM : T_SMEM;
     if (!(configured.load(std::memory_order_acquire) & bit)) {
-        FC_CUDA_OK(cudaFuncSetAttribute(attention_tc_kernel<F16>, cudaFuncAttributeMaxDynamicSharedMemorySize, ACfg<F16>::SMEM));
+        FC_CUDA_OK(cudaFuncSetAttribute(F16 ? attention_tc_f16_kernel : attention_tc_tf32_kernel,
+                                        cudaFuncAttributeMaxDynamicSharedMemorySize, smem));
         configured.fetch_or(bit, std::memory_order_release);
     }
     FcProfScope prof(FC_CLS_ATTENTION, 4.0 * B * (double)N * Nc * d, 4.0 * B * ((double)N * d * 2 + (double)Nc * d * 2), stream);
@@ -557,8 +839,9 @@
     if (dbg_loads < 0) { const char* e = getenv("FC_ATTN_DBG_LOADS"); dbg_loads = (e && e[0] == '1') ? 1 : 0; }
     static int dbg = -1;
     if (dbg < 0) { const char* e = getenv("FC_ATTN_DEBUG"); dbg = (e && e[0] == '1') ? 1 : 0; }
-    AttnTcParams p{out, ldo, N, Nc, (Nc + AK - 1) / AK, scale, dbg, dbg_loads};
-    attention_tc_kernel<F16><<<dim3((N + AQ - 1) / AQ, B), A_THREADS, ACfg<F16>::SMEM, stream>>>(mQ, mKh, mKl, mVh, mVl, p);
+    AttnTcParams p{out, ldo, N, Nc, (Nc + kblk - 1) / kblk, scale, dbg, dbg_loads};
+    (F16 ? attention_tc_f16_kernel : attention_tc_tf32_kernel)<<<dim3((N + AQ - 1) / AQ, B), A_THREADS, smem, stream>>>(
+        mQ, mKh, mKl, mVh, mVl, p);
     fc_count_launch();
     FC_LAUNCH_OK();
     return FC_OK;
diff --git a/flowcompare_b200/csrc/tcgen05.cuh b/flowcompare_b200/csrc/tcgen05.cuh
--- a/flowcompare_b200/csrc/tcgen05.cuh
+++ b/flowcompare_b200/csrc/tcgen05.cuh
@@ -109,6 +109,14 @@
         "tcgen05.mma.cta_group::1.kind::f16 [%0], [%1], %2, %3, p;\n\t"
         "}" ::"r"(tmem_d), "r"(tmem_a), "l"(desc_b), "r"(idesc), "r"(accumulate) : "memory");
 #endif
+}
+__device__ __forceinline__ void umma_f16_ss(uint32_t tmem_d, uint64_t desc_a, uint64_t desc_b, uint32_t idesc, uint32_t accumulate) {
+    asm volatile(
+        "{\n\t"
+        ".reg .pred p;\n\t"
+        "setp.ne.b32 p, %4, 0;\n\t"
+        "tcgen05.mma.cta_group::1.kind::f16 [%0], %1, %2, %3, p;\n\t"
+        "}" ::"r"(tmem_d), "l"(desc_a), "l"(desc_b), "r"(idesc), "r"(accumulate) : "memory");
 }
 __device__ __forceinline__ uint64_t make_kmajor_sw64_desc(uint32_t smem_addr) {
     uint64_t d = 0;
```

Result: no change. 533.0 (median of 6 runs) (+0.4%).
